# liuzuxin/FSRL

Measured on AMD Instinct MI355X. Metric: policy-updates/sec (PPO-Lagrangian update(), SafetyCarCircle-v0 shape, 256x256 MLP, 20k-step buffer), higher is better.
Workload: dtype f32; 1 GPU; configs[1] PPO-Lag update: repeat 4, clip 0.5, KL stop off, batch 256, N=20000 (20x1000), obs 8/act 2, 256x256; seeds_per_gpu=1, parallelism=independent agents x1

## Files before the change

### fsrl_amd/_lib.py

```python
import ctypes as C
import os

_HERE = os.path.dirname(os.path.abspath(__file__))
LIB_PATH = os.environ.get("FSRL_HIP_LIB") or os.path.join(_HERE, "libfsrl_hip.so")

FSRL_OK, FSRL_EINVAL, FSRL_ENOMEM, FSRL_EHIP, FSRL_ESTATE = 0, -22, -12, -5, -1
PPO_NSTATS = 11
ALGO_PPO_LAG, ALGO_TRPO_LAG, ALGO_CPO, ALGO_SAC_LAG, ALGO_FOCOPS = 0, 1, 2, 3, 4


class Config(C.Structure):
    _fields_ = [("algo", C.c_int32), ("obs_dim", C.c_int32), ("act_dim", C.c_int32),
                ("hidden", C.c_int32), ("n_critics", C.c_int32), ("env_num", C.c_int32),
                ("buffer_size", C.c_int64), ("max_action", C.c_float), ("gamma", C.c_double),
                ("gae_lambda", C.c_double), ("eps_clip", C.c_float), ("dual_clip", C.c_float),
                ("vf_coef", C.c_float), ("max_grad_norm", C.c_float), ("target_kl", C.c_float),
                ("norm_adv", C.c_int32), ("use_lagrangian", C.c_int32), ("lr", C.c_float),
                ("beta1", C.c_float), ("beta2", C.c_float), ("adam_eps", C.c_float), ("recompute_adv", C.c_int32),
                ("unbounded", C.c_int32), ("rew_norm", C.c_int32), ("value_clip", C.c_int32),
                ("hidden1", C.c_int32), ("hidden2", C.c_int32),
                ("n_hidden", C.c_int32), ("hidden_sizes", C.c_int32 * 8), ("force_layered", C.c_int32)]


class ShmEnv(C.Structure):
# ... 15 lines not shown
    _fields_ = [("actor_lr", C.c_float), ("critic_lr", C.c_float), ("alpha_lr", C.c_float), ("tau", C.c_float),
                ("alpha", C.c_float), ("target_entropy", C.c_float), ("n_step", C.c_int32),
                ("auto_alpha", C.c_int32), ("use_lagrangian", C.c_int32), ("deterministic", C.c_int32),
                ("exploration_sigma", C.c_float), ("actor_mean", C.c_int32)]


class FocopsConfig(C.Structure):
    _fields_ = [("actor_lr", C.c_float), ("critic_lr", C.c_float), ("l2_reg", C.c_float), ("delta", C.c_float),
                ("eta", C.c_float), ("tem_lambda", C.c_float), ("max_grad_norm", C.c_float)]


class CvpoConfig(C.Structure):
    _fields_ = [("actor_lr", C.c_float), ("critic_lr", C.c_float), ("tau", C.c_float), ("n_step", C.c_int32),
                ("double_critic", C.c_int32), ("sample_act_num", C.c_int32), ("estep_iter_num", C.c_int32),
                ("mstep_iter_num", C.c_int32), ("estep_kl", C.c_float), ("estep_dual_max", C.c_float),
                ("estep_dual_lr", C.c_float), ("mstep_kl_mu", C.c_float), ("mstep_kl_std", C.c_float),
                ("mstep_dual_max", C.c_float), ("mstep_dual_lr", C.c_float), ("qc_thres", C.c_double),
                ("actor_mean", C.c_int32)]


class DevEnvConfig(C.Structure):
    _fields_ = [("kind", C.c_int32), ("env_num", C.c_int32), ("obs_dim", C.c_int32), ("act_dim", C.c_int32),
                ("max_episode_steps", C.c_int32), ("seed", C.c_uint64), ("p", C.c_float * 8), ("A", C.c_void_p), ("B", C.c_void_p)]


DEVENV_POINT_CIRCLE, DEVENV_LINEAR = 0, 1

ACTOR_MEAN_DEFAULT, ACTOR_MEAN_UNBOUNDED, ACTOR_MEAN_TANH = 0, 1, 2


def actor_mean_code(unbounded):
    if unbounded is None:
        return ACTOR_MEAN_DEFAULT
    return ACTOR_MEAN_UNBOUNDED if bool(unbounded) else ACTOR_MEAN_TANH


CPO_NSTATS, TRPO_NSTATS, SAC_NSTATS, FOCOPS_NSTATS, CVPO_NSTATS = 17, 11, 10, 8, 17

_P = C.POINTER
_f, _d, _u8, _i32, _i64 = _P(C.c_float), _P(C.c_double), _P(C.c_uint8), _P(C.c_int32), _P(C.c_int64)
_ctx = C.c_void_p

SIGNATURES = {
    "fsrl_last_error": (C.c_char_p, []),
    "fsrl_config_default": (None, [_P(Config)]),
    "fsrl_mem_live": (C.c_int, [_i64, _i64, _i64, _i64]),
    "fsrl_ctx_create": (C.c_int, [C.c_int, _P(Config), _P(_ctx)]),
    "fsrl_ctx_destroy": (C.c_int, [_ctx]),
    "fsrl_sync": (C.c_int, [_ctx]),
    "fsrl_param_count": (C.c_int64, [_ctx]),
    "fsrl_params_set": (C.c_int, [_ctx, _f, C.c_int64]),
    "fsrl_params_get": (C.c_int, [_ctx, _f, C.c_int64]),
    "fsrl_grads_get": (C.c_int, [_ctx, _f, C.c_int64]),
    "fsrl_optim_reset": (C.c_int, [_ctx]),
    "fsrl_state_snapshot": (C.c_int, [_ctx]),
    "fsrl_state_restore": (C.c_int, [_ctx]),
    "fsrl_train_state_size": (C.c_int64, [_ctx, C.c_int32]),
    "fsrl_train_state_export": (C.c_int, [_ctx, C.c_int32, C.c_void_p, C.c_int64, _i64]),
    "fsrl_train_state_import": (C.c_int, [_ctx, C.c_void_p, C.c_int64]),
    "fsrl_train_state_copy": (C.c_int, [_ctx, _ctx, C.c_int32]),
    "fsrl_ret_rms_get": (C.c_int, [_ctx, _d, C.c_int32]),
    "fsrl_ret_rms_set": (C.c_int, [_ctx, _d, C.c_int32]),
    "fsrl_set_lr": (C.c_int, [_ctx, C.c_int32, C.c_float]),
    "fsrl_get_lr": (C.c_float, [_ctx, C.c_int32]),
    "fsrl_ppo_abort": (C.c_int, [_ctx]),
    "fsrl_store_push": (C.c_int, [_ctx, _i32, C.c_int32, _f, _f, _d, _d, _u8, _u8, _f, _i64, _d, _i32, _i64]),
    "fsrl_store_reset": (C.c_int, [_ctx, C.c_int]),
    "fsrl_store_len": (C.c_int64, [_ctx]),
    "fsrl_store_read": (C.c_int, [_ctx, _i64, C.c_int64, _f, _f, _d, _d, _u8, _u8, _f]),
    "fsrl_store_configure": (C.c_int, [_ctx, C.c_int64, C.c_int32]),
    "fsrl_store_geometry": (C.c_int, [_ctx, _i64, _i32]),
    "fsrl_store_version": (C.c_int, [_ctx, _P(C.c_uint64)]),
    "fsrl_store_sample0": (C.c_int, [_ctx, _i64, C.c_int64, _i64]),
    "fsrl_actor_forward": (C.c_int, [_ctx, _f, C.c_int32, _f, _f]),
    "fsrl_ppo_begin": (C.c_int, [_ctx, _d, C.c_double, C.c_int32, _i64]),
    "fsrl_ppo_pass": (C.c_int, [_ctx, _i64, C.c_uint64, _i32]),
    "fsrl_ppo_pass_result": (C.c_int, [_ctx, _i32]),
    "fsrl_ppo_end": (C.c_int, [_ctx, _f, C.c_int64, _i64]),
    "fsrl_ppo_update": (C.c_int, [_ctx, _d, C.c_double, C.c_int32, C.c_int32, _i64, C.c_uint64, _f,
                                  C.c_int64, _i64, _i32]),
    "fsrl_ppo_set_plan": (C.c_int, [_ctx, C.c_int32]),
    "fsrl_ppo_set_clip_fuse": (C.c_int, [_ctx, C.c_int32, C.c_int32]),
    "fsrl_ppo_clip_fuse_stats": (C.c_int, [_ctx, _i64, _f]),
    "fsrl_batch_get": (C.c_int, [_ctx, C.c_char_p, _f, C.c_int64]),
    "fsrl_group_create": (C.c_int, [_P(_ctx), C.c_int32, _P(_ctx)]),
    "fsrl_group_destroy": (C.c_int, [_ctx]),
    "fsrl_group_set_plan": (C.c_int, [_ctx, C.c_int32]),
    "fsrl_group_ppo_update": (C.c_int, [_ctx, _d, _d, C.c_int32, C.c_int32, _P(_i64), C.c_uint64, _P(_f), C.c_int64, _i64,
                                        _i32]),
    "fsrl_group_ppo_update_each": (C.c_int, [_ctx, _d, _d, _i32, _i32, _P(_i64), C.c_uint64, _P(_f), _i64, _i64, _i32]),
    "fsrl_group_collect_step": (C.c_int, [_ctx, _i32, _i32, _f, _f, _d, _d, _u8, _u8, _f, _i64, _d, _i32, _i64, _i32, _f, C.c_int32,
                                          C.c_int32, _f, _f, _f, _f]),
    "fsrl_group_actor_set_resident": (C.c_int, [_ctx, C.c_int32, C.c_double]),
    "fsrl_group_actor_resident_stats": (C.c_int, [_ctx, _i64]),
    "fsrl_group_actor_release": (C.c_int, [_ctx]),
    "fsrl_sac_group_create": (C.c_int, [_P(_ctx), C.c_int32, _P(_ctx)]),
    "fsrl_sac_group_destroy": (C.c_int, [_ctx]),
    "fsrl_sac_group_update": (C.c_int, [_ctx, C.c_int32, _i32, _d, _d]),
    "fsrl_cvpo_group_create": (C.c_int, [_P(_ctx), C.c_int32, _P(_ctx)]),
    "fsrl_cvpo_group_destroy": (C.c_int, [_ctx]),
    "fsrl_cvpo_group_update": (C.c_int, [_ctx, C.c_int32, _i32]),
    "fsrl_collect_group_create": (C.c_int, [_P(_ctx), C.c_int32, _P(_ctx)]),
    "fsrl_collect_group_destroy": (C.c_int, [_ctx]),
    "fsrl_collect_group_step": (C.c_int, [_ctx, _i32, _i32, _f, _f, _d, _d, _u8, _u8, _f, _i64, _d, _i32, _i64, _i32, _f, C.c_int32,
                                          C.c_int32, _f, _f, _f, _f]),
    "fsrl_collect_group_actor_set_resident": (C.c_int, [_ctx, C.c_int32, C.c_double]),
    "fsrl_collect_group_actor_resident_stats": (C.c_int, [_ctx, _i64]),
    "fsrl_collect_group_actor_release": (C.c_int, [_ctx]),
    "fsrl_group_collect_episodes": (C.c_int, [_ctx, _P(_P(ShmEnv)), _i32, _i32, _f, _i32, C.c_int32, C.c_int32, _f, _f, _i64, _d, _i32,
                                              _i32, _d, _i32, _i32, _d, _i32]),
    "fsrl_collect_episodes_group": (C.c_int, [_ctx, _P(_P(ShmEnv)), _i32, _i32, _f, _i32, C.c_int32, C.c_int32, _f, _f, _i64, _d, _i32,
                                              _i32, _d, _i32, _i32, _d, _i32]),
    "fsrl_gae_return": (C.c_int, [_ctx, _f, _f, _d, _u8, C.c_int64, C.c_double, C.c_double, _d]),
    "fsrl_nstep_return": (C.c_int, [_ctx, _d, _u8, C.c_int64, _f, _i64, C.c_int64, C.c_int64, C.c_double, C.c_int32, _d]),
    "fsrl_launch_floors": (C.c_int, [_ctx, C.c_int32, C.c_int32, _d]),
    "fsrl_tr_begin": (C.c_int, [_ctx, _P(TrConfig), _i64]),
    "fsrl_cpo_learn": (C.c_int, [_ctx, C.c_double, C.c_int32, _f]),
    "fsrl_trpo_learn": (C.c_int, [_ctx, _d, C.c_double, C.c_int32, _f]),
    "fsrl_cpo_learn_mb": (C.c_int, [_ctx, C.c_double, C.c_int32, C.c_int32, _i64, C.c_uint64, _f, C.c_int64, _i64]),
    "fsrl_trpo_learn_mb": (C.c_int, [_ctx, _d, C.c_double, C.c_int32, C.c_int32, _i64, C.c_uint64, _f, C.c_int64, _i64]),
    "fsrl_tr_linesearch_evals": (C.c_int32, [_ctx, _i32, C.c_int32]),
    "fsrl_actor_param_count": (C.c_int64, [_ctx]),
    "fsrl_tr_grad": (C.c_int, [_ctx, C.c_int32, _f, C.c_int64]),
    "fsrl_tr_hvp": (C.c_int, [_ctx, _f, _f, C.c_int64]),
    "fsrl_tr_hvp_cached": (C.c_int, [_ctx, _f, _f, C.c_int64]),
    "fsrl_tr_cg": (C.c_int, [_ctx, _f, C.c_int64, C.c_float, C.c_int32, C.c_float, _f, _i32, _f]),
    "fsrl_tr_eval": (C.c_int, [_ctx, _d]),
    "fsrl_tr_set_plan": (C.c_int, [_ctx, C.c_int32, C.c_int32, C.c_int32]),
    "fsrl_tr_set_tile_split": (C.c_int, [_ctx, C.c_int32, C.c_int32]),
    "fsrl_tr_set_co_delay": (C.c_int, [_ctx, C.c_int32, C.c_int32]),
    "fsrl_focops_init": (C.c_int, [_ctx, _P(FocopsConfig)]),
    "fsrl_focops_set_plan": (C.c_int, [_ctx, C.c_int32]),
    "fsrl_focops_set_nu": (C.c_int, [_ctx, C.c_double, C.c_double]),
    "fsrl_sac_init": (C.c_int, [_ctx, _P(SacConfig)]),
    "fsrl_sac_set_plan": (C.c_int, [_ctx, C.c_int32]),
    "fsrl_sac_param_count": (C.c_int64, [_ctx, C.c_int32]),
    "fsrl_sac_params_set": (C.c_int, [_ctx, _f, C.c_int64, _f, C.c_int64, C.c_float]),
    "fsrl_sac_params_put": (C.c_int, [_ctx, C.c_int32, _f, C.c_int64]),
    "fsrl_sac_params_get": (C.c_int, [_ctx, C.c_int32, _f, C.c_int64, _f]),
    "fsrl_sac_update": (C.c_int, [_ctx, C.c_int32, _i64, _f, _f, C.c_uint64, _d, C.c_double, _f]),
    "fsrl_actor_sample": (C.c_int, [_ctx, _f, C.c_int32, C.c_int32, C.c_uint64, _f]),
    "fsrl_collect_step": (C.c_int, [_ctx, _i32, C.c_int32, _f, _f, _d, _d, _u8, _u8, _f, _i64, _d, _i32, _i64,
                                    _f, C.c_int32, C.c_int32, C.c_int32, _f, _f, _f, _f]),
    "fsrl_collect_episodes": (C.c_int, [_ctx, _P(ShmEnv), _i32, C.c_int32, _f, C.c_int32, C.c_int32, C.c_int32, _f, _f, _i64, _d, _i32,
                                        _i32, _d, _i32, _i32]),
    "fsrl_collect_episodes_split": (C.c_int, [_ctx, _P(ShmEnv), _i32, C.c_int32, _f, C.c_int32, C.c_int32, C.c_int32, _f, _f, _i64, _d, _i32,
                                              _i32, _d, _i32, _i32]),
    "fsrl_collect_timing": (C.c_int, [_ctx, _d]),
    "fsrl_actor_set_resident": (C.c_int, [_ctx, C.c_int32, C.c_double]),
    "fsrl_actor_resident_stats": (C.c_int, [_ctx, _i64]),
    "fsrl_actor_release": (C.c_int, [_ctx]),
    "fsrl_collect_run": (C.c_int, [_ctx, _P(ShmEnv), _i32, C.c_int32, _f, _f, _f, C.c_int32, C.c_int32, _f, _f, C.c_int32, _i32, _d, _d, _d,
                                  _u8, _u8, _f]),
    "fsrl_store_sizes": (C.c_int, [_ctx, _i64, C.c_int32]),
    "fsrl_sac_stats_drain": (C.c_int64, [_ctx, _f, C.c_int64]),
    "fsrl_sac_last_sample": (C.c_int, [_ctx, _i64, _f, _f, C.c_int32]),
    "fsrl_sac_last_chain": (C.c_int, [_ctx, _i64, _u8, C.c_int32]),
    "fsrl_per_enable": (C.c_int, [_ctx, C.c_double, C.c_double, C.c_int32]),
    "fsrl_per_set_beta": (C.c_int, [_ctx, C.c_double]),
    "fsrl_per_update_weight": (C.c_int, [_ctx, _i64, _d, C.c_int64]),
    "fsrl_per_state": (C.c_int, [_ctx, _d, C.c_int64, _d, _d, _d]),
    "fsrl_per_last_weights": (C.c_int, [_ctx, _f, C.c_int32]),
    "fsrl_per_last_td": (C.c_int, [_ctx, _f, C.c_int32]),
    "fsrl_sac_actor_forward": (C.c_int, [_ctx, _f, C.c_int32, _f, _f]),
    "fsrl_cvpo_init": (C.c_int, [_ctx, _P(CvpoConfig)]),
    "fsrl_cvpo_pre_update": (C.c_int, [_ctx]),
# ... 86 lines not shown
```

### fsrl_amd/csrc/fsrl_hip.hip

```cpp
#include <hip/hip_runtime.h>

#include <climits>
#include <cstddef>
#include <cmath>
#include <cstdarg>
#include <cstdio>
#include <cstdlib>
#include <cstring>
#include <algorithm>
#include <functional>
#include <string>
#include <vector>

#include <atomic>
#include "kernels_misc.hpp"
#include "kernels_mlp.hpp"
#include "kernels_fb.hpp"
#include "kernels_fbco.hpp"
#include "kernels_wgrad2.hpp"
#include "kernels_wgrad3.hpp"
#include "kernels_layered.hpp"
#include "kernels_focops_group.hpp"
#include "resident_ring.hpp"
#include "host_decisions.hpp"
// ... 6 lines not shown
    va_start(ap, fmt);
    vsnprintf(buf, sizeof(buf), fmt, ap);
    va_end(ap);
    g_err = buf;
    return code;
}
#define HIPCHK(expr)                                                                        \
    do {                                                                                    \
        hipError_t _e = (expr);                                                             \
        if (_e != hipSuccess)                                                               \
            return fail(FSRL_EHIP, "%s failed: %s (%s:%d)", #expr, hipGetErrorString(_e),   \
                        __FILE__, __LINE__);                                                \
    } while (0)
#define CHECK_ARG(cond, ...) \
    do { if (!(cond)) return fail(FSRL_EINVAL, __VA_ARGS__); } while (0)

extern "C" const char* fsrl_last_error(void) { return g_err.c_str(); }

static inline int round_up(int x, int m) { return (x + m - 1) / m * m; }

struct TensorMap {
    int api_off, dev_off, rows, cols, dev_ld;
    int n() const { return rows * cols; }
    void to_dev(float* dev, const float* api) const {
        for (int r = 0; r < rows; ++r) memcpy(dev + dev_off + (size_t)r * dev_ld, api + api_off + (size_t)r * cols, (size_t)cols * 4);
    }
    void to_api(float* api, const float* dev) const {
        for (int r = 0; r < rows; ++r) memcpy(api + api_off + (size_t)r * cols, dev + dev_off + (size_t)r * dev_ld, (size_t)cols * 4);
    }
};

struct EnvBook {
    int64_t index = 0, size = 0, last_index = 0;
    int64_t staged = 0;
    double ep_rew = 0.0;
    int32_t ep_len = 0;
    int64_t ep_idx = 0;
};

struct Staging {
    uint8_t* h = nullptr;
    uint8_t* d = nullptr;
    int count = 0;
    hipEvent_t done = nullptr;
    bool in_flight = false;
};
static inline size_t stage_rec_bytes(int Do, int Da) { return ((size_t)24 + 4 * (size_t)(2 * Do + Da) + 7) / 8 * 8; }

struct fsrl_group;
struct fsrl_ctx {
    fsrl_config cfg{};
    Mem mem;
    fsrl_group* group = nullptr;
    struct CommState* comm = nullptr;
    int device = 0;
    hipStream_t compute = nullptr, side = nullptr;
    ModelDesc md{};
    std::vector<TensorMap> tmap;
    int h1 = 0, h2 = 0;
    int64_t n_api = 0;
    int n_dev = 0;
    int n_alloc = 0;
    float *P = nullptr, *M = nullptr, *V = nullptr, *G = nullptr;
    int64_t adam_t = 0;
    CtrlBlock* ctrl = nullptr;
    CtrlBlock* h_ctrl = nullptr;
    bool verdict_pending = false;

    int64_t sub_size = 0, maxsize = 0;
    float* mbstat = nullptr; size_t mbstat_cap = 0;
    double* d_rms = nullptr;
    double* ret64 = nullptr; int64_t ret64_cap = 0;
    int64_t alloc_rows = 0;
    int active_envs = 0;
    std::vector<EnvBook> env;
    std::vector<uint8_t> h_flags;
    StorePtrs st{};
    static constexpr int STAGE_CAP = 4096;
    Staging stage[2];
    int cur_stage = 0;
    hipEvent_t store_ready = nullptr;

    BatchPtrs b{};
    int* d_indices = nullptr; uint8_t* d_end = nullptr; int* d_seg = nullptr;
    int* h_indices = nullptr; uint8_t* h_end = nullptr; int* h_seg = nullptr;
    float *values = nullptr, *vnext = nullptr, *advs = nullptr, *rets = nullptr, *logp_old = nullptr;
    int64_t N = 0;
    int n_seg = 0;
    bool batch_ready = false;

    int batch_size = 0, mbp_max = 0, n_tiles_max = 0;
    float *A1 = nullptr, *A2 = nullptr, *D1 = nullptr, *D2 = nullptr, *DO = nullptr;
    float *obs_p = nullptr, *rd_p = nullptr;
    float *statp = nullptr, *gsq_part = nullptr;
    int *d_perm = nullptr, *h_perm = nullptr;
    int *d_mbstart = nullptr, *d_mbsize = nullptr, *h_mbplan = nullptr;
    size_t mb_cap = 0;
    std::vector<int> mb_start, mb_size;
    float* d_stats = nullptr; int64_t stats_cap = 0;
    int64_t n_steps = 0;
    int pass_index = 0;
    double lagr[FSRL_MAX_CRITICS] = {0, 0, 0, 0};
    double rescaling = 1.0;
    bool in_update = false;

    void* scratch = nullptr; size_t scratch_bytes = 0;

    bool profiling = false;
    hipEvent_t ev_a = nullptr, ev_b = nullptr, ev_c = nullptr;
    std::vector<hipEvent_t> k_ev;
    size_t k_ev_used = 0;
    double t_process_ms = 0, t_learn_ms = 0, t_fwdbwd_ms = 0, t_fwdbwd_raw_ms = 0;
    int64_t n_fwdbwd = 0;
    uint64_t rng[4] = {0x9E3779B97F4A7C15ull, 0xBF58476D1CE4E5B9ull, 0x94D049BB133111EBull, 1};
    uint64_t shuffle_rng[4] = {0xD6E8FEB86659FD93ull, 0xA0761D6478BD642Full, 0xE7037ED1A0B428DBull, 2};
    struct Parts { int stride = 0; float* p = nullptr; size_t floats = 0; } parts[3];
    float* wg_parts = nullptr;
    int n_cus = 256;
    bool wgrad_xcd = false;
    bool wgrad_stream = false;
    int wgrad_tiles = 1;
    struct FocState* foc = nullptr;
    float* mu_old = nullptr;
    float* sigma_old = nullptr;
    void* h_actor = nullptr; size_t h_actor_bytes = 0;
    int actor_k = 0; size_t actor_ob = 0, actor_mb = 0;
    unsigned* h_done = nullptr; int done_cap = 0;
    unsigned actor_seq = 0; int actor_blocks = 0;
    ResidentRing pa;
    bool pa_req = false;
    int pa_cap = 0;
    void* h_pa = nullptr;
    int probe_phase = 0, probe_wgrad_skip = 0;
    unsigned long long* probe_ts = nullptr;
    bool probe_tile16 = false;
    struct fsrl_sac_group* sac_group = nullptr;
    struct fsrl_cvpo_group* cvpo_group = nullptr;
    struct fsrl_collect_group* cgroup = nullptr;
    int tall_tiles = -1;
    bool no_fuse_adam = false;
    bool no_w2b_early = false;
    bool counted_live = false;
    int clip_fuse_mode = -1;
    int clip_fuse_limit = CLIP_FUSE_DEFAULT_TICKS;
    bool no_clip_fuse = false;
    bool clip_fuse_dead = false;
    bool clip_fuse_active = false;
    int64_t clip_fuse_fallbacks = 0, clip_fuse_steps = 0;
    unsigned clip_epoch = 0;
    unsigned long long* clip_slots = nullptr;
    float* clip_snap = nullptr;
    int64_t clip_snap_adam_t = 0;
    std::vector<std::vector<int>> clip_perms;
    bool no_xcd_pair = false;
    bool no_spin = false;
    std::vector<float> act_mu, act_sg;
    std::vector<int> perm_tmp;
    hipEvent_t perm_copied = nullptr; bool perm_in_flight = false;
    uint64_t store_version = 1;
    uint64_t joined_version = 0;
    double t_collect_env = 0.0, t_collect_act = 0.0;
    float* snap = nullptr;
    int64_t snap_adam_t = 0, snap_critic_t = 0, snap_foc_a = 0, snap_foc_c = 0; bool snap_valid = false;
    struct LayState* lay = nullptr;
    struct TrState* tr = nullptr;
    uint64_t theta_version = 1;
    void* sac = nullptr;
    struct fsrl_tap* tap = nullptr;
    struct PerState* per = nullptr;
    std::vector<struct fsrl_devenv*> devenvs;
};
static bool ctx_is_replay(const fsrl_ctx* c);
static void sac_free(fsrl_ctx* c);
static void tr_free(fsrl_ctx* c);
static void foc_free(fsrl_ctx* c);
static void tr_reset_optim(fsrl_ctx* c);
static int64_t tr_critic_steps_taken(fsrl_ctx* c);
static void tr_set_critic_steps(fsrl_ctx* c, int64_t t);
static void foc_steps(fsrl_ctx* c, int64_t* t_actor, int64_t* t_critic, bool set);
static void foc_reset_optim(fsrl_ctx* c);
static void group_detach(fsrl_ctx* c);
static void lay_free(fsrl_ctx* c);
static void lay_build_layout(fsrl_ctx* c, const int* widths, int L);
static int lay_ensure_mb(fsrl_ctx* c, int B);
static int lay_ppo_steps(fsrl_ctx* c);
struct InferArgs;
static int lay_infer(fsrl_ctx* c, const InferArgs& ia, int jobs_y, hipStream_t s);
static void comm_free(fsrl_ctx* c);
static inline bool tap_closed(const fsrl_ctx* c, int e);
static void tap_row(fsrl_ctx* c, int e, int i, const float* act, double rew, double cost, uint8_t fl);
static int tap_flush(fsrl_ctx* c, int w, const uint8_t* recs_d, int stage_rec, int k);
static void tap_ctx_gone(fsrl_ctx* c);
static void devenv_ctx_gone(fsrl_ctx* c);
static int per_ingest(fsrl_ctx* c, const uint8_t* recs_d, int rec, int k);
static int per_store_reset(fsrl_ctx* c);
static void per_free(fsrl_ctx* c);
static int focops_pass(fsrl_ctx* c, int32_t* stopped_out);
static int pass_verdict(fsrl_ctx* c, int32_t* stopped_out);

static int flush_stage(fsrl_ctx* c);
static void pactor_release(fsrl_ctx* c);
static void group_actor_release(fsrl_group* g);
static void sac_group_detach(fsrl_ctx* c);
static void cvpo_group_detach(fsrl_ctx* c);
static void collect_group_detach(fsrl_ctx* c);
static void collect_group_actor_release(struct fsrl_collect_group* g);
static int focops_group_check(fsrl_ctx* const* ctxs, int k);
struct GroupUpdate;
static int focops_group_update(GroupUpdate& u);
#define ENTER_DEV(c) do { HIPCHK(hipSetDevice((c)->device)); pactor_release(c); } while (0)

static int join_store(fsrl_ctx* c) {
    if (c->joined_version == c->store_version) return 0;
    int rc = flush_stage(c);
    if (rc) return rc;
    HIPCHK(hipEventRecord(c->store_ready, c->side));
    HIPCHK(hipStreamWaitEvent(c->compute, c->store_ready, 0));
    c->joined_version = c->store_version;
    return 0;
}

static int ensure_scratch(fsrl_ctx* c, size_t bytes) {
    HIPCHK(c->mem.regrow(c->scratch_bytes, bytes, bytes, {Mem::D(&c->scratch, bytes)}));
    return 0;
}

template <class T>
struct DevTable { T *d = nullptr, *h = nullptr; size_t cap = 0; };
template <class T>
static int table_ensure(DevTable<T>& t, size_t need, size_t grow_to, hipStream_t sync = nullptr) {
    if (need <= t.cap) return 0;
    if (sync) HIPCHK(hipStreamSynchronize(sync));
    const size_t old = t.cap * sizeof(T);
    t.cap = 0;
// ... 196 lines not shown
    if (c->sac_group) sac_group_detach(c);
    if (c->cvpo_group) cvpo_group_detach(c);
    if (c->cgroup) collect_group_detach(c);
    devenv_ctx_gone(c);
    if (c->tap) tap_ctx_gone(c);
    comm_free(c);
    tr_free(c);
    sac_free(c);
    per_free(c);
    foc_free(c);
    lay_free(c);
    c->mem.release_all();
    for (auto& st : c->stage) if (st.done) (void)hipEventDestroy(st.done);
    for (hipEvent_t e : {c->store_ready, c->ev_a, c->ev_b, c->ev_c, c->perm_copied}) if (e) (void)hipEventDestroy(e);
    for (hipEvent_t e : c->k_ev) (void)hipEventDestroy(e);
    if (c->compute) (void)hipStreamDestroy(c->compute);
    if (c->side) (void)hipStreamDestroy(c->side);
    if (c->counted_live && c->device >= 0 && c->device < 64) g_live_ctx[c->device].fetch_sub(1);
    delete c;
    return 0;
}

extern "C" int fsrl_ctx_create(int device_id, const fsrl_config* cfg, fsrl_ctx** out) {
    CHECK_ARG(cfg && out, "null argument");
    CHECK_ARG(cfg->algo == FSRL_ALGO_PPO_LAG || cfg->algo == FSRL_ALGO_SAC_LAG || cfg->algo == FSRL_ALGO_CPO ||
                  cfg->algo == FSRL_ALGO_TRPO_LAG || cfg->algo == FSRL_ALGO_FOCOPS, "unknown algo %d", cfg->algo);
    CHECK_ARG(cfg->obs_dim >= 1 && cfg->obs_dim <= FSRL_MAX_OBS, "obs_dim must be in [1,%d]", FSRL_MAX_OBS);
    CHECK_ARG(cfg->act_dim >= 1 && cfg->act_dim <= FSRL_MAX_ACT, "act_dim must be in [1,%d]", FSRL_MAX_ACT);
    CHECK_ARG(cfg->n_hidden >= 0 && cfg->n_hidden <= FSRL_MAX_HIDDEN, "n_hidden must be in [0, %d]", FSRL_MAX_HIDDEN);
    bool layered = false;
    int n_hid1 = cfg->hidden1, n_hid2 = cfg->hidden2;
    if (cfg->n_hidden > 0) {
        CHECK_ARG(cfg->hidden1 == 0 && cfg->hidden2 == 0, "give hidden_sizes[n_hidden] or hidden1 / hidden2, not both");
        for (int l = 0; l < cfg->n_hidden; ++l)
            CHECK_ARG(cfg->hidden_sizes[l] >= 1 && cfg->hidden_sizes[l] <= FSRL_MAX_WIDTH, "hidden_sizes[%d] = %d outside [1, %d]", l,
                      cfg->hidden_sizes[l], FSRL_MAX_WIDTH);
        if (cfg->n_hidden == 2 && cfg->hidden_sizes[0] <= 256 && cfg->hidden_sizes[1] <= 256 && !cfg->force_layered) {
            n_hid1 = cfg->hidden_sizes[0]; n_hid2 = cfg->hidden_sizes[1];
        } else {
            layered = true;
        }
    } else {
        CHECK_ARG(!cfg->force_layered, "force_layered needs hidden_sizes[n_hidden]");
    }
    const int h1_ = layered ? 0 : (n_hid1 > 0 ? n_hid1 : cfg->hidden), h2_ = layered ? 0 : (n_hid2 > 0 ? n_hid2 : cfg->hidden);
    if (!layered) {
        CHECK_ARG((n_hid1 > 0) == (n_hid2 > 0), "hidden1 and hidden2 are given together (0, 0 = two layers of `hidden`)");
        CHECK_ARG(h1_ >= 1 && h1_ <= 256 && h2_ >= 1 && h2_ <= 256, "hidden layer widths must be in [1, 256] (two hidden layers)");
    }
    const int Hpad_ = layered ? 0 : std::max(h1_, h2_) <= 64 ? 64 : std::max(h1_, h2_) <= 128 ? 128 : 256;
    CHECK_ARG(layered || n_hid1 == 0 || cfg->hidden == 0 || cfg->hidden == Hpad_ ,
              "hidden = %d does not fit hidden1 / hidden2 = %d / %d (leave hidden 0 or give %d)", cfg->hidden, h1_, h2_, Hpad_);
    CHECK_ARG(!layered || cfg->n_critics < 1 || cfg->n_critics > FSRL_MAX_CRITICS ||
                  (1 + cfg->n_critics) * (cfg->n_hidden + 1) + 1 <= LAY_MAX_JOBS,
              "layered context: (1 + n_critics) * (n_hidden + 1) + 1 = %d weight-gradient jobs exceed the job table of %d "
              "(n_critics = %d, n_hidden = %d)", (1 + cfg->n_critics) * (cfg->n_hidden + 1) + 1, LAY_MAX_JOBS, cfg->n_critics, cfg->n_hidden);
    CHECK_ARG(cfg->n_critics >= 1 && cfg->n_critics <= 2,
              "n_critics must be 1 or 2 (reward [+ one cost], get_metrics base_policy.py:377-382)");
    CHECK_ARG(cfg->env_num >= 1 && cfg->buffer_size >= cfg->env_num, "bad env_num/buffer_size");
    CHECK_ARG(cfg->gamma >= 0.0 && cfg->gamma <= 1.0, "discount factor should be in [0, 1].");
    CHECK_ARG(cfg->gae_lambda >= 0.0 && cfg->gae_lambda <= 1.0, "GAE lambda should be in [0, 1].");
    CHECK_ARG(cfg->dual_clip == 0.0f || cfg->dual_clip > 1.0f,
              "Dual-clip PPO parameter should greater than 1.0.");
    CHECK_ARG(cfg->buffer_size + cfg->env_num < (int64_t)INT_MAX / 2, "buffer too large for 32-bit slot ids");
    CHECK_ARG(cfg->rew_norm || !cfg->value_clip, "value clip is available only when `reward_normalization` is True");
    CHECK_ARG(!cfg->value_clip || cfg->algo == FSRL_ALGO_PPO_LAG, "value_clip is a PPO-Lagrangian option (ppo_lag.py:158-164)");
    CHECK_ARG(!cfg->rew_norm || cfg->algo != FSRL_ALGO_SAC_LAG, "reward_normalization acts on GAE returns: on-policy contexts only");
    int ndev = 0;
    HIPCHK(hipGetDeviceCount(&ndev));
    CHECK_ARG(device_id >= 0 && device_id < ndev, "device %d not present (%d devices)", device_id, ndev);
    HIPCHK(hipSetDevice(device_id));
    int n_cus_probe = 256;
    (void)hipDeviceGetAttribute(&n_cus_probe, hipDeviceAttributeMultiprocessorCount, device_id);
    fsrl_ctx* c = new fsrl_ctx();
    c->cfg = *cfg;
    c->cfg.hidden = Hpad_;
    c->h1 = h1_; c->h2 = h2_;
    c->device = device_id;
    if (device_id >= 0 && device_id < 64) { g_live_ctx[device_id].fetch_add(1); c->counted_live = true; }
    c->n_cus = n_cus_probe > 0 ? n_cus_probe : 256;
    c->probe_tile16 = getenv("FSRL_TILE16") != nullptr;
    c->no_w2b_early = getenv("FSRL_NO_W2B_EARLY") != nullptr;
    c->no_clip_fuse = getenv("FSRL_NO_CLIP_FUSE") != nullptr;
#ifdef FSRL_PROBES
    { const char* e = getenv("FSRL_DBG_PHASE"); c->probe_phase = e ? atoi(e) : 0; }
    { const char* e = getenv("FSRL_WGRAD_SKIP"); c->probe_wgrad_skip = e ? atoi(e) : 0; }
    c->no_spin = getenv("FSRL_NO_SPIN") != nullptr;
    c->no_xcd_pair = getenv("FSRL_NO_XCD_PAIR") != nullptr;
    c->no_fuse_adam = getenv("FSRL_NO_FUSE_ADAM") != nullptr;
    if (getenv("FSRL_TSTAMP")) {
        if (c->mem.dev(&c->probe_ts, 1024 * 16 * sizeof(unsigned long long)) == hipSuccess)
            (void)hipMemset(c->probe_ts, 0, 1024 * 16 * sizeof(unsigned long long));
    }
#endif
    if (layered) lay_build_layout(c, cfg->hidden_sizes, cfg->n_hidden);
    else build_layout(c);
#define TRY(expr) do { hipError_t _e = (expr); if (_e != hipSuccess) { fail(FSRL_EHIP, "%s failed: %s", #expr, hipGetErrorString(_e)); fsrl_ctx_destroy(c); return FSRL_EHIP; } } while (0)
    TRY(hipStreamCreateWithFlags(&c->compute, hipStreamNonBlocking));
    TRY(hipStreamCreateWithFlags(&c->side, hipStreamNonBlocking));
    const size_t pb = (size_t)c->n_dev * sizeof(float);
    TRY(c->mem.dev(&c->P, (size_t)c->n_alloc * sizeof(float))); TRY(hipMemsetAsync(c->P, 0, (size_t)c->n_alloc * sizeof(float), c->compute));
    TRY(c->mem.dev(&c->M, pb)); TRY(c->mem.dev(&c->V, pb)); TRY(c->mem.dev(&c->G, pb));
    TRY(hipMemsetAsync(c->M, 0, pb, c->compute)); TRY(hipMemsetAsync(c->V, 0, pb, c->compute)); TRY(hipMemsetAsync(c->G, 0, pb, c->compute));
    TRY(c->mem.dev(&c->ctrl, sizeof(CtrlBlock)));
    if (cfg->rew_norm) {
        TRY(c->mem.dev(&c->d_rms, 3 * FSRL_MAX_CRITICS * sizeof(double)));
        double init[3 * FSRL_MAX_CRITICS];
        for (int i = 0; i < FSRL_MAX_CRITICS; ++i) { init[3 * i] = 0.0; init[3 * i + 1] = 1.0; init[3 * i + 2] = 0.0; }
        TRY(hipMemcpy(c->d_rms, init, sizeof(init), hipMemcpyHostToDevice));
    }
    TRY(c->mem.pinned(&c->h_ctrl, sizeof(CtrlBlock)));
    c->sub_size = (cfg->buffer_size + cfg->env_num - 1) / cfg->env_num;
    c->maxsize = c->sub_size * cfg->env_num;
    c->alloc_rows = c->maxsize + cfg->env_num; c->active_envs = cfg->env_num;
    c->env.resize(cfg->env_num);
    c->h_flags.assign((size_t)c->alloc_rows, 0);
    const size_t ms = (size_t)c->alloc_rows;
    const int Do = cfg->obs_dim, Da = cfg->act_dim;
    TRY(c->mem.dev(&c->st.obs, ms * Do * 4)); TRY(c->mem.dev(&c->st.obs_next, ms * Do * 4));
    TRY(c->mem.dev(&c->st.act, ms * Da * 4)); TRY(c->mem.dev(&c->st.rew, ms * 8));
    TRY(c->mem.dev(&c->st.cost, ms * 8)); TRY(c->mem.dev(&c->st.flags, ms));
    TRY(c->mem.dev(&c->b.obs, ms * Do * 4)); TRY(c->mem.dev(&c->b.obs_next, ms * Do * 4));
    TRY(c->mem.dev(&c->b.act, ms * Da * 4)); TRY(c->mem.dev(&c->b.rew, ms * 8));
    TRY(c->mem.dev(&c->b.cost, ms * 8)); TRY(c->mem.dev(&c->b.flags, ms));
    TRY(c->mem.dev(&c->d_indices, ms * 4)); TRY(c->mem.dev(&c->d_end, ms)); TRY(c->mem.dev(&c->d_seg, (ms + 2) * 4));
    TRY(c->mem.pinned(&c->h_indices, ms * 4)); TRY(c->mem.pinned(&c->h_end, ms)); TRY(c->mem.pinned(&c->h_seg, (ms + 2) * 4));
    const int C = cfg->n_critics;
    TRY(c->mem.dev(&c->values, ms * C * 4)); TRY(c->mem.dev(&c->vnext, ms * C * 4));
    TRY(c->mem.dev(&c->advs, ms * C * 4)); TRY(c->mem.dev(&c->rets, ms * C * 4));
    TRY(c->mem.dev(&c->logp_old, ms * 4));
    TRY(c->mem.dev(&c->d_perm, ms * 4)); TRY(c->mem.pinned(&c->h_perm, ms * 4));
    TRY(c->mem.dev(&c->obs_p, (ms + 32) * Do * 4)); TRY(hipMemsetAsync(c->obs_p, 0, (ms + 32) * Do * 4, c->compute));
    TRY(c->mem.dev(&c->rd_p, (ms + 32) * FSRL_RD * 4)); TRY(hipMemsetAsync(c->rd_p, 0, (ms + 32) * FSRL_RD * 4, c->compute));
    TRY(hipStreamSynchronize(c->compute));
    for (auto& s : c->stage) {
        const size_t k = fsrl_ctx::STAGE_CAP;
        TRY(c->mem.pinned(&s.h, k * stage_rec_bytes(Do, Da)));
        TRY(c->mem.dev(&s.d, k * stage_rec_bytes(Do, Da)));
        TRY(hipEventCreateWithFlags(&s.done, hipEventDisableTiming));
    }
    TRY(hipEventCreateWithFlags(&c->store_ready, hipEventDisableTiming));
    TRY(hipEventCreate(&c->ev_a)); TRY(hipEventCreate(&c->ev_b)); TRY(hipEventCreate(&c->ev_c));
    TRY(hipEventCreateWithFlags(&c->perm_copied, hipEventDisableTiming));
    CtrlBlock init{INT_MAX, 0, 0.0, 0.0f, 0.0f};
    TRY(hipMemcpy(c->ctrl, &init, sizeof(init), hipMemcpyHostToDevice));
#undef TRY
    *out = c;
    return 0;
}

extern "C" int fsrl_sync(fsrl_ctx* c) {
    CHECK_ARG(c, "null ctx");
    ENTER_DEV(c);
    HIPCHK(hipStreamSynchronize(c->side));
    HIPCHK(hipStreamSynchronize(c->compute));
    return 0;
}

extern "C" int64_t fsrl_param_count(const fsrl_ctx* c) { return c ? c->n_api : 0; }

static int copy_flat(fsrl_ctx* c, float* dev, float* host_out, const float* host_in, int64_t n) {
    CHECK_ARG(n == c->n_api, "expected %lld parameters, got %lld", (long long)c->n_api, (long long)n);
    ENTER_DEV(c);
    std::vector<float> tmp((size_t)c->n_dev, 0.0f);
    if (host_in) {
        for (const TensorMap& t : c->tmap) t.to_dev(tmp.data(), host_in);
        HIPCHK(hipStreamSynchronize(c->compute));
        HIPCHK(hipMemcpy(dev, tmp.data(), (size_t)c->n_dev * 4, hipMemcpyHostToDevice));
        hipLaunchKernelGGL(w2f_sync_kernel, dim3(192), dim3(256), 0, c->compute, dev, c->md);
        HIPCHK(hipGetLastError());
    } else {
        HIPCHK(hipStreamSynchronize(c->compute));
        HIPCHK(hipMemcpy(tmp.data(), dev, (size_t)c->n_dev * 4, hipMemcpyDeviceToHost));
        for (const TensorMap& t : c->tmap) t.to_api(host_out, tmp.data());
    }
    return 0;
}

extern "C" int fsrl_params_set(fsrl_ctx* c, const float* flat, int64_t n) {
    CHECK_ARG(c && flat, "null argument");
    c->theta_version += 1;
    return copy_flat(c, c->P, nullptr, flat, n);
}
extern "C" int fsrl_params_get(fsrl_ctx* c, float* flat, int64_t n) {
    CHECK_ARG(c && flat, "null argument");
    return copy_flat(c, c->P, flat, nullptr, n);
}
extern "C" int fsrl_grads_get(fsrl_ctx* c, float* flat, int64_t n) {
    CHECK_ARG(c && flat, "null argument");
    return copy_flat(c, c->G, flat, nullptr, n);
}
extern "C" int fsrl_optim_reset(fsrl_ctx* c) {
    CHECK_ARG(c, "null ctx");
    ENTER_DEV(c);
    HIPCHK(hipStreamSynchronize(c->compute));
    HIPCHK(hipMemsetAsync(c->M, 0, (size_t)c->n_dev * 4, c->compute));
    HIPCHK(hipMemsetAsync(c->V, 0, (size_t)c->n_dev * 4, c->compute));
    HIPCHK(hipStreamSynchronize(c->compute));
    c->adam_t = 0;
    tr_reset_optim(c);
    foc_reset_optim(c);
    return 0;
}

extern "C" int fsrl_state_snapshot(fsrl_ctx* c) {
    CHECK_ARG(c, "null ctx");
    CHECK_ARG(!c->in_update, "fsrl_state_snapshot inside an update");
    CHECK_ARG(!ctx_is_replay(c), "fsrl_state_snapshot covers on-policy contexts (PPO-Lag, FOCOPS, CPO, TRPO-Lag) only");
    ENTER_DEV(c);
// ... 178 lines not shown
        for (int64_t i = eb.index; i < eb.size; ++i) idx[n++] = (int)(off + i);
        for (int64_t i = 0; i < eb.index; ++i) idx[n++] = (int)(off + i);
        if (endf) {
            for (int64_t r = first; r < n; ++r) endf[r] = c->h_flags[(size_t)idx[r]] != 0;
            if (n > first) endf[n - 1] = 1;
        }
    }
    return n;
}

extern "C" int fsrl_store_sample0(fsrl_ctx* c, int64_t* out, int64_t cap, int64_t* n_out) {
    CHECK_ARG(c && n_out, "null argument");
    const int64_t n = sample0(c, c->h_indices, nullptr);
    *n_out = n;
    if (out) {
        CHECK_ARG(cap >= n, "indices_out too small (%lld < %lld)", (long long)cap, (long long)n);
        for (int64_t i = 0; i < n; ++i) out[i] = c->h_indices[i];
    }
    return 0;
}

extern "C" int fsrl_store_read(fsrl_ctx* c, const int64_t* indices, int64_t n, float* obs_out, float* act_out,
                               double* rew_out, double* cost_out, uint8_t* terminated_out, uint8_t* truncated_out,
                               float* obs_next_out) {
    CHECK_ARG(c && (indices || n == 0), "null argument");
    CHECK_ARG(n >= 0 && n <= c->maxsize, "bad row count");
    if (n == 0) return 0;
    ENTER_DEV(c);
    int rc = join_store(c);
    if (rc) return rc;
    const size_t N = (size_t)n, Do = (size_t)c->cfg.obs_dim, Da = (size_t)c->cfg.act_dim;
    auto al = [](size_t x) { return (x + 255) / 256 * 256; };
    const size_t o_idx = 0, o_end = o_idx + al(N * 4), o_obs = o_end + al(N), o_nxt = o_obs + al(N * Do * 4),
                 o_act = o_nxt + al(N * Do * 4), o_rew = o_act + al(N * Da * 4), o_cost = o_rew + al(N * 8),
                 o_fl = o_cost + al(N * 8), total = o_fl + al(N);
    rc = ensure_scratch(c, total);
    if (rc) return rc;
    std::vector<int> idx(N);
    for (size_t i = 0; i < N; ++i) {
        CHECK_ARG(indices[i] >= 0 && indices[i] < c->maxsize, "index %lld out of range", (long long)indices[i]);
        idx[i] = (int)indices[i];
    }
    char* base = (char*)c->scratch;
    hipStream_t s = c->compute;
    HIPCHK(hipMemcpyAsync(base + o_idx, idx.data(), N * 4, hipMemcpyHostToDevice, s));
    HIPCHK(hipMemsetAsync(base + o_end, 0, N, s));
    BatchPtrs b{(float*)(base + o_obs), (float*)(base + o_nxt), (float*)(base + o_act), (double*)(base + o_rew),
                (double*)(base + o_cost), (uint8_t*)(base + o_fl)};
    const size_t work = N * (2 * Do + Da + 1);
    hipLaunchKernelGGL(batch_gather_kernel, dim3((int)std::min<size_t>(2048, (work + 255) / 256)), dim3(256), 0, s, c->st, b,
                       (const int*)(base + o_idx), (const uint8_t*)(base + o_end), (int)n, (int)Do, (int)Da);
    HIPCHK(hipGetLastError());
    std::vector<uint8_t> fl(N);
    if (obs_out) HIPCHK(hipMemcpyAsync(obs_out, b.obs, N * Do * 4, hipMemcpyDeviceToHost, s));
    if (obs_next_out) HIPCHK(hipMemcpyAsync(obs_next_out, b.obs_next, N * Do * 4, hipMemcpyDeviceToHost, s));
    if (act_out) HIPCHK(hipMemcpyAsync(act_out, b.act, N * Da * 4, hipMemcpyDeviceToHost, s));
    if (rew_out) HIPCHK(hipMemcpyAsync(rew_out, b.rew, N * 8, hipMemcpyDeviceToHost, s));
    if (cost_out) HIPCHK(hipMemcpyAsync(cost_out, b.cost, N * 8, hipMemcpyDeviceToHost, s));
    HIPCHK(hipMemcpyAsync(fl.data(), b.flags, N, hipMemcpyDeviceToHost, s));
    HIPCHK(hipStreamSynchronize(s));
    for (size_t i = 0; i < N; ++i) {
        if (terminated_out) terminated_out[i] = fl[i] & 1;
        if (truncated_out) truncated_out[i] = (fl[i] >> 1) & 1;
    }
    return 0;
}

template <typename F>
static int dispatch_H(int H, F&& f) {
    switch (H) {
        case 64: return f(std::integral_constant<int, 64>());
        case 128: return f(std::integral_constant<int, 128>());
        case 256: return f(std::integral_constant<int, 256>());
    }
    return fail(FSRL_EINVAL, "unsupported hidden width %d", H);
}

static int launch_infer(fsrl_ctx* c, const InferArgs& ia, int jobs_y, hipStream_t s) {
    const int tiles = (ia.N + 15) / 16;
    if (tiles == 0) return 0;
    if (c->lay) return lay_infer(c, ia, jobs_y, s);
    return dispatch_H(c->cfg.hidden, [&](auto hc) {
        constexpr int H = decltype(hc)::value;
        const int gx = std::min(tiles, std::max(1, c->n_cus / jobs_y));
        hipLaunchKernelGGL(mlp_infer_kernel<H>, dim3(gx, jobs_y), dim3(4 * H), 0, s, c->P, c->md, ia);
        HIPCHK(hipGetLastError());
        return 0;
    });
}

struct SacState;
static bool ctx_is_replay(const fsrl_ctx* c) { return c->cfg.algo == FSRL_ALGO_SAC_LAG; }
static int sac_actor_launch(fsrl_ctx* c, const float* h_obs, float* h_raw, int k);
static void sac_actor_finish(fsrl_ctx* c, const float* h_raw, int k, float* mu_out, float* sigma_out);
static int sac_raw_cols(const fsrl_ctx* c);
static bool sac_squashes(fsrl_ctx* c);
static bool sac_actor_resident_args(fsrl_ctx* c, const float** P, const ModelDesc** md);

struct PaLayout { unsigned long long* bell; unsigned* done; unsigned* state; float* obs; float* mu; float* sp; };
static PaLayout pa_layout(const fsrl_ctx* c) {
    char* b = (char*)c->h_pa;
    PaLayout l;
    l.bell = (unsigned long long*)b; l.done = (unsigned*)(b + 16); l.state = (unsigned*)(b + 32);
    l.obs = (float*)(b + 64);
    l.mu = l.obs + (size_t)c->pa_cap * c->cfg.obs_dim;
    l.sp = l.mu + (size_t)c->pa_cap * 2 * c->cfg.act_dim;
    return l;
}

static bool pactor_ok(const fsrl_ctx* c, int k) {
    const int blocks = std::min(PACTOR_BLOCKS, std::max(1, (c->cfg.env_num + 15) / 16));
    if (!(c->pa.on && !c->no_spin && !c->lay && !c->group && k >= 1 && k <= 16 * blocks)) return false;
    if (c->cfg.algo != FSRL_ALGO_SAC_LAG) return true;
    const float* P; const ModelDesc* md;
    return sac_actor_resident_args(const_cast<fsrl_ctx*>(c), &P, &md);
}

static void pactor_release(fsrl_ctx* c) {
    if (c->group) group_actor_release(c->group);
    if (c->cgroup) collect_group_actor_release(c->cgroup);
    rr_release(c->pa);
}

static int stream_state(hipStream_t s) {
    const hipError_t e = hipStreamQuery(s);
    if (e == hipSuccess || e == hipErrorNotReady) return e == hipSuccess ? RR_STREAM_IDLE : RR_STREAM_BUSY;
    fail(FSRL_EHIP, "the resident actor's stream: %s", hipGetErrorString(e));
    return RR_STREAM_ERROR;
}
static int rr_code(int rc, const char* what) {
    if (rc <= 0) return rc;
    if (rc == RR_ERROR) return FSRL_EHIP;
    if (rc == RR_BAD_TIMEOUT) return fail(FSRL_EINVAL, "idle_timeout_us above one second");
    return fail(FSRL_EHIP, "%s does not answer", what);
}

static int pactor_launch(void* owner, ResidentRing& r, unsigned last_seq) {
    fsrl_ctx* c = (fsrl_ctx*)owner;
    const PaLayout l = pa_layout(c);
    PActorArgs a{};
    a.obs = l.obs; a.mu_out = l.mu; a.sigma_param_out = l.sp; a.bell = l.bell; a.done = l.done; a.state = l.state;
    a.gen = r.gen; a.last_seq = last_seq; a.max_action = c->cfg.max_action;
    a.timeout_ticks = (unsigned long long)(r.idle_us * 100.0);
    r.blocks = r.tiles[0] = std::min(PACTOR_BLOCKS, std::max(1, (c->cfg.env_num + 15) / 16));
    const float* P = c->P; const ModelDesc* md = &c->md;
    if (c->cfg.algo == FSRL_ALGO_SAC_LAG) {
        if (!sac_actor_resident_args(c, &P, &md)) return fail(FSRL_ESTATE, "no fused actor network");
        a.raw_cols = sac_raw_cols(c); a.max_action = 1.0f;
    }
    const ModelDesc mdv = *md;
    return dispatch_H(c->cfg.hidden, [&](auto hc) {
        constexpr int H = decltype(hc)::value;
        if (a.raw_cols > 0) hipLaunchKernelGGL((actor_resident_kernel<H, true>), dim3(r.blocks), dim3(4 * H), 0, c->compute, P, mdv, a);
        else hipLaunchKernelGGL((actor_resident_kernel<H, false>), dim3(r.blocks), dim3(4 * H), 0, c->compute, P, mdv, a);
        HIPCHK(hipGetLastError());
        return 0;
    });
}

static int pactor_post(fsrl_ctx* c, const float* obs, int k) {
    const int Do = c->cfg.obs_dim, Da = c->cfg.act_dim;
    ResidentRing& r = c->pa;
    if (!c->h_pa) {
        const int cap = 16 * PACTOR_BLOCKS;
        const size_t bytes = 64 + ((size_t)cap * (Do + 2 * Da) + FSRL_MAX_ACT) * 4;
        HIPCHK(c->mem.regrow(c->pa_cap, cap, cap, {Mem::H(&c->h_pa, bytes)}));
        memset(c->h_pa, 0, bytes);
// ... 445 lines not shown
```

### fsrl_amd/csrc/host_decisions.hpp

```cpp
#pragma once
#include <stdint.h>
#include <algorithm>
#include <cmath>
#include <functional>
#include <queue>
#include <vector>

static constexpr float CPO_EPS = 1e-8f;
static inline bool cpo_cost_solve_skipped(float bb, float c_value) { return bb <= CPO_EPS && c_value < 0; }
struct CpoDual { int ocase; float A, B, lam, nu; };
static inline CpoDual cpo_dual_solve(float s_q, float s_r, float s_s, float c_value, float delta, float bb) {
    const float EPS = CPO_EPS;
    float A = 0.f, B = 0.f, lam, nu;
    int ocase = 4;
    if (!cpo_cost_solve_skipped(bb, c_value)) {
        A = s_q - s_r * s_r / s_s;
        B = 2.0f * delta - c_value * c_value / s_s;
        if (c_value < 0 && B < 0) ocase = 3;
        else if (c_value < 0 && B >= 0) ocase = 2;
        else if (c_value >= 0 && B >= 0) ocase = 1;
        else ocase = 0;
    }
    if (ocase == 3 || ocase == 4) {
        lam = std::sqrt(s_q / (2.0f * delta));
// ... 60 lines not shown
static inline uint64_t rotl64(uint64_t x, int k) { return (x << k) | (x >> (64 - k)); }
static inline uint64_t xoshiro_next(uint64_t* s) {
    const uint64_t result = rotl64(s[1] * 5, 7) * 9, t = s[1] << 17;
    s[2] ^= s[0]; s[3] ^= s[1]; s[1] ^= s[2]; s[0] ^= s[3]; s[2] ^= t; s[3] = rotl64(s[3], 45);
    return result;
}
enum { PERM_OK = 0, PERM_RANGE, PERM_TWICE };
struct PermFill { int code, index; long long value; };
static inline PermFill perm_fill(int* out, int n, const int64_t* perm, uint64_t* rng, uint64_t seed) {
    if (perm) {
        std::vector<uint8_t> seen((size_t)n, 0);
        for (int i = 0; i < n; ++i) {
            if (!(perm[i] >= 0 && perm[i] < n)) return {PERM_RANGE, i, (long long)perm[i]};
            if (seen[(size_t)perm[i]]) return {PERM_TWICE, i, (long long)perm[i]};
            seen[(size_t)perm[i]] = 1;
            out[i] = (int)perm[i];
        }
        return {PERM_OK, 0, 0};
    }
    if (seed) { rng[0] ^= seed; rng[1] += seed * 0x9E3779B97F4A7C15ull; }
    for (int i = 0; i < n; ++i) out[i] = i;
    for (int i = n - 1; i > 0; --i) std::swap(out[i], out[(int)(xoshiro_next(rng) % (uint64_t)(i + 1))]);
    return {PERM_OK, 0, 0};
}

struct TileSplit { int n32, n16; };
static inline TileSplit mixed_split(int64_t N, int ny, int n_cus, double rho) {
    const int max32 = (int)((N + 31) / 32);
    double best = 1e300; int best32 = 0, best16 = (int)((N + 15) / 16);
    std::vector<double> cu((size_t)std::max(n_cus, 1));
    for (int n32 = 0; n32 <= max32; ++n32) {
        const int64_t rem = N - 32 * (int64_t)n32;
        const int n16 = rem > 0 ? (int)((rem + 15) / 16) : 0;
        if (n16 > 0 && n32 == max32) continue;
        std::fill(cu.begin(), cu.end(), 0.0);
        std::priority_queue<double, std::vector<double>, std::greater<double>> pq(cu.begin(), cu.end());
        double span = 0.0;
        for (int b = 0; b < ny * n32; ++b) { const double e = pq.top() + 1.0; pq.pop(); pq.push(e); span = std::max(span, e); }
        for (int b = 0; b < ny * n16; ++b) { const double e = pq.top() + rho; pq.pop(); pq.push(e); span = std::max(span, e); }
        if (span < best - 1e-9 || (std::fabs(span - best) <= 1e-9 && n32 > best32)) { best = span; best32 = n32; best16 = n16; }
    }
    return {best32, best16};
}
static inline void co_plan(int64_t N, int n_wgs, int* n32_out, int* n16_out) {
    const int64_t tail_rows = std::min<int64_t>(N, 16 * (int64_t)(n_wgs / 2));
    const int n32 = (int)((N - tail_rows) / 32);
    const int64_t rem = N - 32 * (int64_t)n32;
    *n32_out = n32; *n16_out = (int)((rem + 15) / 16);
}
static inline void forced_split(int64_t N, int want32, int* n32_out, int* n16_out) {
    const int n32 = (int)std::min<int64_t>(want32, N / 32);
    const int64_t rem = N - 32 * (int64_t)n32;
    *n32_out = n32; *n16_out = (int)((rem + 15) / 16);
}

static constexpr int CLIP_FUSE_DEFAULT_TICKS = 5000;
static constexpr int CLIP_FUSE_MAX_OBS = 64;
struct ClipFuseFacts {
    int mode;
    bool env_off;
    bool dead;
    bool ppo_lag, layered, grouped;
    bool recompute_adv, rew_norm;
    float max_grad_norm;
    int nparts, n_cus;
    int obs_dim;
    int live_contexts;
};
static inline bool clip_fuse_update_ok(const ClipFuseFacts& f) {
    if (f.mode == 0 || f.env_off || f.dead) return false;
    if (f.mode < 0 && f.live_contexts > 1) return false;
    if (!f.ppo_lag || f.layered || f.grouped) return false;
    if (!(f.max_grad_norm > 0.0f)) return false;
    if (f.recompute_adv || f.rew_norm) return false;
    if (f.nparts > f.n_cus || f.nparts > 1024) return false;
    return f.obs_dim <= CLIP_FUSE_MAX_OBS;
}
static inline bool clip_fuse_step_ok(bool update_ok, int rows_pad) { return update_ok && rows_pad <= 512; }
static inline bool clip_fuse_must_replay(bool active, int poisoned) { return active && poisoned != 0; }
struct ClipFuseReplay { long long adam_t, n_steps; int pass_index, passes; };
static inline ClipFuseReplay clip_fuse_replay_plan(long long snap_adam_t, int passes_enqueued) {
    return {snap_adam_t, 0, 0, passes_enqueued};
}
```

### fsrl_amd/csrc/host_ppo.inc

```
static int launch_gae(fsrl_ctx* c);
static int perm_send(fsrl_ctx* c, int n);
static int clip_fuse_begin(fsrl_ctx* c);
static int perm_upload(fsrl_ctx* c, int n, const int64_t* perm, uint64_t seed) {
    c->perm_tmp.resize((size_t)n);
    const PermFill pf = perm_fill(c->perm_tmp.data(), n, perm, c->shuffle_rng, seed);
    CHECK_ARG(pf.code != PERM_RANGE, "perm[%d]=%lld out of range", pf.index, pf.value);
    CHECK_ARG(pf.code != PERM_TWICE, "perm is not a permutation: %lld appears twice", pf.value);
    return perm_send(c, n);
}
static int perm_send(fsrl_ctx* c, int n) {
    if (c->perm_in_flight) { HIPCHK(hipEventSynchronize(c->perm_copied)); c->perm_in_flight = false; }
    memcpy(c->h_perm, c->perm_tmp.data(), (size_t)n * 4);
    HIPCHK(hipMemcpyAsync(c->d_perm, c->h_perm, (size_t)n * 4, hipMemcpyHostToDevice, c->compute));
    HIPCHK(hipEventRecord(c->perm_copied, c->compute));
    c->perm_in_flight = true;
    return 0;
}

static int ensure_ppo_buffers(fsrl_ctx* c, int B) {
    const int mbp = round_up(2 * B, 32);
    if (mbp <= c->mbp_max) return 0;
    HIPCHK(hipStreamSynchronize(c->compute));
    const int H = c->cfg.hidden, nn = c->md.n_nets;
    const size_t act = (size_t)nn * mbp * H * 4;
    HIPCHK(c->mem.regrow(c->mbp_max, mbp, mbp,
                         {Mem::D(&c->A1, act), Mem::D(&c->A2, act), Mem::D(&c->D1, act), Mem::D(&c->D2, act),
                          Mem::D(&c->DO, (size_t)nn * mbp * FSRL_DOW * 4),
                          Mem::D(&c->statp, (size_t)(mbp / 4) * nn * 4 * 4),
                          Mem::D(&c->gsq_part, (size_t)std::max(wg_grid(H, nn), c->n_dev / 256 + 2) * 4)}));
    c->n_tiles_max = mbp / 16;
    return 0;
}

extern "C" int fsrl_ppo_set_plan(fsrl_ctx* c, int32_t tall_tiles) {
    CHECK_ARG(c, "null ctx");
    CHECK_ARG(tall_tiles >= -1 && tall_tiles <= 4096, "tall_tiles: -1 (automatic), 0 (none) or a count");
    c->tall_tiles = tall_tiles;
    return 0;
}

extern "C" int fsrl_ppo_begin(fsrl_ctx* c, const double* lagrangians, double rescaling,
                              int32_t batch_size, int64_t* n_out) {
    CHECK_ARG(c, "null ctx");
    CHECK_ARG(batch_size >= 1, "batch_size must be >= 1");
    CHECK_ARG(!c->in_update, "fsrl_ppo_begin called twice without fsrl_ppo_end");
    ENTER_DEV(c);
    int rc = flush_stage(c);
    if (rc) return rc;
    HIPCHK(hipEventRecord(c->store_ready, c->side));
    HIPCHK(hipStreamWaitEvent(c->compute, c->store_ready, 0));
    const int C = c->cfg.n_critics;
    for (int i = 0; i < FSRL_MAX_CRITICS; ++i) c->lagr[i] = 0.0;
    if (c->cfg.use_lagrangian && C > 1) {
        CHECK_ARG(lagrangians, "lags and values length must be equal");
        for (int i = 0; i < C - 1; ++i) c->lagr[i] = lagrangians[i];
    }
    c->rescaling = rescaling;
    c->batch_size = batch_size;
    const int64_t n = sample0(c, c->h_indices, c->h_end);
    c->N = n;
    if (n_out) *n_out = n;
    c->n_steps = 0;
    c->pass_index = 0;
    c->in_update = true;
    c->verdict_pending = false;
    c->t_fwdbwd_ms = 0; c->n_fwdbwd = 0; c->k_ev_used = 0;
    CtrlBlock init{INT_MAX, 0, 0.0, 0.0f, 0.0f};
    *c->h_ctrl = init;
    hipStream_t s = c->compute;
    HIPCHK(hipMemcpyAsync(c->ctrl, c->h_ctrl, sizeof(CtrlBlock), hipMemcpyHostToDevice, s));
    c->clip_fuse_active = false;
    c->clip_perms.clear();
    if (n == 0) { c->batch_ready = true; return 0; }
    rc = clip_fuse_begin(c);
    if (rc) return rc;
    int nseg = 0;
    c->h_seg[nseg++] = 0;
    for (int64_t i = 0; i + 1 < n; ++i) if (c->h_end[i]) c->h_seg[nseg++] = (int)i + 1;
    c->h_seg[nseg] = (int)n;
    HIPCHK(hipEventRecord(c->ev_a, s));
    HIPCHK(hipMemcpyAsync(c->d_indices, c->h_indices, (size_t)n * 4, hipMemcpyHostToDevice, s));
    HIPCHK(hipMemcpyAsync(c->d_end, c->h_end, (size_t)n, hipMemcpyHostToDevice, s));
    HIPCHK(hipMemcpyAsync(c->d_seg, c->h_seg, (size_t)(nseg + 1) * 4, hipMemcpyHostToDevice, s));
    const int Do = c->cfg.obs_dim, Da = c->cfg.act_dim;
    {
        const size_t work = (size_t)n * (2 * Do + Da + 1);
        const int blocks = (int)std::min<size_t>(2048, (work + 255) / 256);
        hipLaunchKernelGGL(batch_gather_kernel, dim3(blocks), dim3(256), 0, s, c->st, c->b, c->d_indices,
                           c->d_end, (int)n, Do, Da);
        HIPCHK(hipGetLastError());
    }
    InferArgs ia{};
    ia.obs = c->b.obs; ia.obs_next = c->b.obs_next; ia.act = c->b.act; ia.flags = c->b.flags;
    ia.values = c->values; ia.vnext = c->vnext; ia.logp_old = c->logp_old; ia.mu_out = nullptr;
    if (c->cfg.algo == FSRL_ALGO_FOCOPS) {
        if (!c->mu_old) {
            HIPCHK(c->mem.dev(&c->mu_old, (size_t)c->alloc_rows * Da * 4));
            HIPCHK(c->mem.dev(&c->sigma_old, FSRL_MAX_ACT * 4));
        }
        ia.mu_out = c->mu_old;
        HIPCHK(hipMemcpyAsync(c->sigma_old, c->P + c->md.net[0].sigma, (size_t)Da * 4, hipMemcpyDeviceToDevice, s));
    }
    ia.N = (int)n; ia.C = C; ia.max_action = c->cfg.max_action;
    rc = launch_infer(c, ia, 2 * C + 1, s);
    if (rc) return rc;
    c->n_seg = nseg;
    rc = launch_gae(c);
    if (rc) return rc;
    HIPCHK(hipEventRecord(c->ev_b, s));
    split_plan((int)n, batch_size, c->mb_start, c->mb_size);
    const int bs_rows = (int)std::min<int64_t>(batch_size, std::max<int64_t>(n, 1));
    rc = c->lay ? lay_ensure_mb(c, bs_rows) : ensure_ppo_buffers(c, bs_rows);
    if (rc) return rc;
    const size_t nmb = c->mb_start.size();
    if (nmb > c->mb_cap) {
        HIPCHK(hipStreamSynchronize(s));
        const size_t cap = nmb * 2;
        HIPCHK(c->mem.regrow(c->mb_cap, nmb, cap, {Mem::D(&c->d_mbstart, cap * 4), Mem::D(&c->d_mbsize, cap * 4), Mem::H(&c->h_mbplan, cap * 2 * 4)}));
    }
    memcpy(c->h_mbplan, c->mb_start.data(), nmb * 4);
    memcpy(c->h_mbplan + c->mb_cap, c->mb_size.data(), nmb * 4);
    HIPCHK(hipMemcpyAsync(c->d_mbstart, c->h_mbplan, nmb * 4, hipMemcpyHostToDevice, s));
    HIPCHK(hipMemcpyAsync(c->d_mbsize, c->h_mbplan + c->mb_cap, nmb * 4, hipMemcpyHostToDevice, s));
    c->batch_ready = true;
    return 0;
}


static int launch_gae(fsrl_ctx* c) {
    GaeArgs ga{};
    ga.values = c->values; ga.vnext = c->vnext; ga.rew = c->b.rew; ga.cost = c->b.cost; ga.flags = c->b.flags;
    ga.seg_start = c->d_seg; ga.advs = c->advs; ga.rets = c->rets; ga.adv64 = nullptr; ga.N = (int)c->N;
    ga.gamma = c->cfg.gamma; ga.gl = c->cfg.gamma * c->cfg.gae_lambda;
    if (c->cfg.rew_norm) {
        if (c->ret64_cap < c->N) {
            HIPCHK(hipStreamSynchronize(c->compute));
            HIPCHK(c->mem.regrow(c->ret64_cap, c->N, c->alloc_rows, {Mem::D(&c->ret64, (size_t)c->cfg.n_critics * c->alloc_rows * 8)}));
        }
        ga.rms = c->d_rms; ga.ret64 = c->ret64;
    }
    hipLaunchKernelGGL(gae_kernel, dim3(c->n_seg, c->cfg.n_critics), dim3(64), 0, c->compute, ga);
    HIPCHK(hipGetLastError());
    if (c->cfg.rew_norm) {
        hipLaunchKernelGGL(ret_rms_update_kernel, dim3(c->cfg.n_critics), dim3(1024), 0, c->compute, c->ret64, c->d_rms,
                           (int)c->N);
        HIPCHK(hipGetLastError());
    }
    return 0;
}

static int ppo_recompute_advantages(fsrl_ctx* c) {
    const int C = c->cfg.n_critics;
    InferArgs ia{};
    ia.obs = c->b.obs; ia.obs_next = c->b.obs_next; ia.act = nullptr; ia.flags = c->b.flags;
    ia.values = c->values; ia.vnext = c->vnext; ia.logp_old = nullptr; ia.mu_out = nullptr;
    ia.N = (int)c->N; ia.C = C; ia.max_action = c->cfg.max_action;
    int rc = launch_infer(c, ia, 2 * C, c->compute);
    if (rc) return rc;
    return launch_gae(c);
}

static int ensure_stats(fsrl_ctx* c, int64_t steps) {
    if (steps <= c->stats_cap) return 0;
    int64_t cap = std::max<int64_t>(steps, c->stats_cap * 2);
    cap = std::max<int64_t>(cap, 1024);
    float* nw = nullptr;
    HIPCHK(c->mem.dev(&nw, (size_t)cap * FSRL_PPO_NSTATS * 4));
    if (c->d_stats) {
        HIPCHK(hipStreamSynchronize(c->compute));
        HIPCHK(hipMemcpy(nw, c->d_stats, (size_t)c->stats_cap * FSRL_PPO_NSTATS * 4, hipMemcpyDeviceToDevice));
        HIPCHK(c->mem.release(&c->d_stats));
    }
    c->d_stats = nw;
    c->stats_cap = cap;
    return 0;
}

static int ppo_pass_prepare(fsrl_ctx* c, const int64_t* perm, uint64_t seed, const std::vector<int>* kept = nullptr) {
    const int n = (int)c->N;
    hipStream_t s = c->compute;
    const int C = c->cfg.n_critics;
    if (c->cfg.recompute_adv && c->pass_index > 0 &&
        (c->cfg.algo == FSRL_ALGO_PPO_LAG || c->cfg.algo == FSRL_ALGO_FOCOPS)) {
        int rc0 = ppo_recompute_advantages(c);
        if (rc0) return rc0;
    }
    int rc;
    if (kept) { c->perm_tmp = *kept; rc = perm_send(c, n); }
    else rc = perm_upload(c, n, perm, seed);
    if (rc) return rc;
    if (c->clip_fuse_active && !kept) c->clip_perms.push_back(c->perm_tmp);
    const int nmb = (int)c->mb_start.size();
    rc = ensure_stats(c, c->n_steps + nmb);
    if (rc) return rc;
    {
        PrepArgs pa{};
        pa.obs = c->b.obs; pa.act = c->b.act; pa.advs = c->advs; pa.rets = c->rets; pa.logp_old = c->logp_old;
        pa.perm = c->d_perm; pa.mb_start = c->d_mbstart; pa.mb_size = c->d_mbsize; pa.obs_p = c->obs_p;
        pa.rd_p = c->rd_p; pa.N = n; pa.C = C; pa.Do = c->cfg.obs_dim; pa.Da = c->cfg.act_dim;
        pa.norm_adv = c->cfg.norm_adv;
        pa.values = c->cfg.value_clip ? c->values : nullptr;
        pa.mean_old = (c->cfg.algo == FSRL_ALGO_FOCOPS) ? c->mu_old : nullptr; pa.sigma_old = c->sigma_old;
        if ((size_t)nmb > c->mbstat_cap) {
            HIPCHK(hipStreamSynchronize(s));
            HIPCHK(c->mem.regrow(c->mbstat_cap, (size_t)nmb, (size_t)nmb * 2, {Mem::D(&c->mbstat, (size_t)nmb * 2 * FSRL_MAX_CRITICS * 2 * sizeof(float))}));
        }
        pa.mbstat = c->mbstat; pa.batch = c->mb_size[0]; pa.nmb = nmb;
        if (pa.norm_adv) hipLaunchKernelGGL(ppo_adv_stats_kernel, dim3(nmb), dim3(1024), 0, s, pa);
        hipLaunchKernelGGL(ppo_permute_rows_kernel, dim3((n + 63) / 64), dim3(256), 0, s, pa);
        HIPCHK(hipGetLastError());
    }
    return 0;
}

static PpoStepArgs ppo_base_args(const fsrl_ctx* c) {
    PpoStepArgs sa{};
    sa.rescale = (float)c->rescaling;
    for (int i = 0; i < FSRL_MAX_CRITICS; ++i) sa.lam[i] = (float)c->lagr[i];
    sa.eps_clip = c->cfg.eps_clip; sa.dual_clip = c->cfg.dual_clip; sa.vf_coef = c->cfg.vf_coef;
    sa.max_action = c->cfg.max_action; sa.max_grad_norm = c->cfg.max_grad_norm; sa.target_kl = c->cfg.target_kl;
    sa.norm_adv = c->cfg.norm_adv; sa.use_lagrangian = c->cfg.use_lagrangian;
    sa.value_clip = c->cfg.value_clip;
    sa.lr = c->cfg.lr; sa.beta1 = c->cfg.beta1; sa.beta2 = c->cfg.beta2; sa.adam_eps = c->cfg.adam_eps;
    sa.one_minus_b1 = (float)(1.0 - (double)c->cfg.beta1);
    sa.one_minus_b2 = (float)(1.0 - (double)c->cfg.beta2);
    sa.kl_thresh = 1.5 * (double)c->cfg.target_kl;
    sa.pass = c->pass_index;
    sa.dbg_phase = c->probe_phase;
    sa.fuse_adam = (c->cfg.max_grad_norm <= 0.0f && !c->no_fuse_adam) ? 1 : 0;
    return sa;
}

static PpoBatchPtrs ppo_batch_ptrs(const fsrl_ctx* c) {
    PpoBatchPtrs bp{};
    bp.obs_p = c->obs_p; bp.rd_p = c->rd_p; bp.A1 = c->A1; bp.A2 = c->A2; bp.D1 = c->D1; bp.D2 = c->D2;
    bp.DO = c->DO; bp.statp = c->statp; bp.mbp_max = c->mbp_max;
    bp.ts = c->probe_ts;
    return bp;
}
// ... 94 lines not shown
                hipEvent_t e; HIPCHK(hipEventCreate(&e)); c->k_ev.push_back(e);
            }
            HIPCHK(hipEventRecord(c->k_ev[c->k_ev_used], s));
        }
        const PpoTilePlan tp = ppo_tile_plan(c, tiles, nn, 1, c->tall_tiles);
        const int n32 = tp.n32, stat_tiles = tp.rows4 ? tiles * 4 : tp.rows8 ? tiles * 2 : tiles;
        rc = dispatch_H(H, [&](auto hc) {
            constexpr int HH = decltype(hc)::value;
            sa.xcd_pair = (nn <= 4 && !c->no_xcd_pair) ? 1 : 0;
            auto fb_grid = [&](int nt) { return sa.xcd_pair ? dim3(8 * ((nt + 1) / 2)) : dim3(nt * nn); };
            const bool early = !c->no_w2b_early;
            if (tp.rows4 && early) hipLaunchKernelGGL((ppo_fwd_bwd_kernel<HH, 4, true>), fb_grid(tiles * 4), dim3(4 * HH), 0, s, c->P, c->md, bp, sa);
            else if (tp.rows4) hipLaunchKernelGGL((ppo_fwd_bwd_kernel<HH, 4>), fb_grid(tiles * 4), dim3(4 * HH), 0, s, c->P, c->md, bp, sa);
            else if (tp.rows8 && early) hipLaunchKernelGGL((ppo_fwd_bwd_kernel<HH, 8, true>), fb_grid(tiles * 2), dim3(4 * HH), 0, s, c->P, c->md, bp, sa);
            else if (tp.rows8) hipLaunchKernelGGL((ppo_fwd_bwd_kernel<HH, 8>), fb_grid(tiles * 2), dim3(4 * HH), 0, s, c->P, c->md, bp, sa);
            else if (n32 > 0) {
                if constexpr (HH >= 128)
                    hipLaunchKernelGGL((ppo_fwd_bwd_tall_kernel<HH>), dim3((tiles - n32) * nn), dim3(4 * HH), 0, s, c->P, c->md, bp, sa, n32, tiles - n32);
            } else hipLaunchKernelGGL((ppo_fwd_bwd_kernel<HH, 16>), fb_grid(tiles), dim3(4 * HH), 0, s, c->P, c->md, bp, sa);
            return 0;
        });
        if (rc) return rc;
        if (prof) {
            HIPCHK(hipEventRecord(c->k_ev[c->k_ev_used + 1], s));
            HIPCHK(hipEventRecord(c->k_ev[c->k_ev_used + 2], s));
            c->k_ev_used += 3;
        }
        const bool big = tiles * 16 > 512;
        const bool clip_step = clip_fuse_step_ok(c->clip_fuse_active, tiles * 16);
        if (clip_step) {
            c->clip_epoch += 1;
            if (c->clip_epoch == 0) c->clip_epoch = 1;
            sa.clip_epoch = c->clip_epoch; sa.clip_limit = c->clip_fuse_limit;
            c->clip_fuse_steps += 1;
        }
        if (big) {
            FbWgradArgs wa{};
            wgrad_fill_nets(wa, nn, 0, (size_t)H, (size_t)c->mbp_max, c->A1, c->A2, c->D1, c->D2, c->DO);
            wa.obs = wp.X; wa.rows = tiles * 16; wa.N = sa.mb_size;
            int nsplit = 1;
            rc = wgrad_launch<false>(c, c->md, wa, nn, c->n_dev, &nsplit);
            if (rc) return rc;
            const int nsum = (c->n_dev + 255) / 256;
            hipLaunchKernelGGL(fb_sum_parts_kernel, dim3(nsum), dim3(256), 0, s, c->G, c->wg_parts, 0, c->n_dev, nsplit, c->n_dev,
                               c->gsq_part);
            hipLaunchKernelGGL(ppo_stats_kernel, dim3(1), dim3(64), 0, s, c->md, wp, sa, stat_tiles);
            hipLaunchKernelGGL(adam_clip_kernel, dim3((c->n_dev + 4 * ADAM_NT - 1) / (4 * ADAM_NT)), dim3(ADAM_NT), 0, s, c->P, c->M,
                               c->V, c->G, c->gsq_part, nsum, c->n_dev, sa, c->ctrl, c->md);
            HIPCHK(hipGetLastError());
            continue;
        }
        rc = dispatch_H(H, [&](auto hc) {
            constexpr int HH = decltype(hc)::value;
            if (sa.fuse_adam) hipLaunchKernelGGL((ppo_wgrad_kernel<HH, false, true>), dim3(nparts), dim3(1024), 0, s, c->md, wp, tiles * 16, sa, stat_tiles);
            else if (clip_step) hipLaunchKernelGGL((ppo_wgrad_kernel<HH, false, true, true>), dim3(nparts), dim3(1024), 0, s, c->md, wp, tiles * 16, sa, stat_tiles);
            else hipLaunchKernelGGL((ppo_wgrad_kernel<HH, false, false>), dim3(nparts), dim3(1024), 0, s, c->md, wp, tiles * 16, sa, stat_tiles);
            return 0;
        });
        if (rc) return rc;
        if (!sa.fuse_adam && !clip_step)
            hipLaunchKernelGGL(adam_clip_kernel, dim3((c->n_dev + 4 * ADAM_NT - 1) / (4 * ADAM_NT)), dim3(ADAM_NT), 0, s, c->P, c->M, c->V, c->G,
                               c->gsq_part, nparts, c->n_dev, sa, c->ctrl, c->md);
        HIPCHK(hipGetLastError());
    }
    c->n_steps += nmb;
    c->pass_index += 1;
    return 0;
}

static int clip_fuse_begin(fsrl_ctx* c) {
    ClipFuseFacts f{};
    f.mode = c->clip_fuse_mode; f.env_off = c->no_clip_fuse; f.dead = c->clip_fuse_dead;
    f.ppo_lag = c->cfg.algo == FSRL_ALGO_PPO_LAG; f.layered = c->lay != nullptr; f.grouped = c->group != nullptr;
    f.recompute_adv = c->cfg.recompute_adv != 0; f.rew_norm = c->cfg.rew_norm != 0;
    f.max_grad_norm = c->cfg.max_grad_norm;
    f.nparts = c->lay ? 0 : wg_grid(c->cfg.hidden, c->md.n_nets); f.n_cus = c->n_cus; f.obs_dim = c->cfg.obs_dim;
    f.live_contexts = live_contexts_on(c->device);
    if (!clip_fuse_update_ok(f)) return 0;
    hipStream_t s = c->compute;
    if (!c->clip_slots) {
        HIPCHK(c->mem.dev(&c->clip_slots, (size_t)1024 * CLIP_SLOT_STRIDE * sizeof(unsigned long long)));
        HIPCHK(hipMemsetAsync(c->clip_slots, 0, (size_t)1024 * CLIP_SLOT_STRIDE * sizeof(unsigned long long), s));
    }
    if (!c->clip_snap) HIPCHK(c->mem.dev(&c->clip_snap, ((size_t)c->n_alloc + 2 * (size_t)c->n_dev) * 4));
    HIPCHK(hipMemcpyAsync(c->clip_snap, c->P, (size_t)c->n_alloc * 4, hipMemcpyDeviceToDevice, s));
    HIPCHK(hipMemcpyAsync(c->clip_snap + c->n_alloc, c->M, (size_t)c->n_dev * 4, hipMemcpyDeviceToDevice, s));
    HIPCHK(hipMemcpyAsync(c->clip_snap + c->n_alloc + c->n_dev, c->V, (size_t)c->n_dev * 4, hipMemcpyDeviceToDevice, s));
    c->clip_snap_adam_t = c->adam_t;
    c->clip_fuse_active = true;
    return 0;
}
static int clip_fuse_check(fsrl_ctx* c) {
    if (!clip_fuse_must_replay(c->clip_fuse_active, c->h_ctrl->poisoned)) return 0;
    hipStream_t s = c->compute;
    const ClipFuseReplay rp = clip_fuse_replay_plan(c->clip_snap_adam_t, c->pass_index);
    c->clip_fuse_active = false; c->clip_fuse_dead = true;
    c->clip_fuse_fallbacks += 1;
    HIPCHK(hipMemcpyAsync(c->P, c->clip_snap, (size_t)c->n_alloc * 4, hipMemcpyDeviceToDevice, s));
    HIPCHK(hipMemcpyAsync(c->M, c->clip_snap + c->n_alloc, (size_t)c->n_dev * 4, hipMemcpyDeviceToDevice, s));
    HIPCHK(hipMemcpyAsync(c->V, c->clip_snap + c->n_alloc + c->n_dev, (size_t)c->n_dev * 4, hipMemcpyDeviceToDevice, s));
    c->adam_t = rp.adam_t; c->n_steps = rp.n_steps; c->pass_index = rp.pass_index;
    c->k_ev_used = 0;
    CtrlBlock init{INT_MAX, 0, 0.0, 0.0f, 0.0f};
    *c->h_ctrl = init;
    HIPCHK(hipMemcpyAsync(c->ctrl, c->h_ctrl, sizeof(CtrlBlock), hipMemcpyHostToDevice, s));
    HIPCHK(hipStreamSynchronize(s));
    for (int k = 0; k < rp.passes; ++k) {
        int rc = ppo_pass_enqueue(c, nullptr, 0, &c->clip_perms[(size_t)k]);
        if (rc) return rc;
    }
    HIPCHK(hipMemcpyAsync(c->h_ctrl, c->ctrl, sizeof(CtrlBlock), hipMemcpyDeviceToHost, s));
    HIPCHK(hipStreamSynchronize(s));
    c->clip_perms.clear();
    return 0;
}
extern "C" int fsrl_ppo_set_clip_fuse(fsrl_ctx* c, int32_t mode, int32_t limit_ticks) {
    CHECK_ARG(c, "null ctx");
    CHECK_ARG(mode >= -1 && mode <= 1, "mode: -1 (automatic), 0 (off) or 1 (on)");
    CHECK_ARG(limit_ticks <= 100000000, "limit_ticks: at most 10^8 (one second)");
    CHECK_ARG(!c->in_update, "fsrl_ppo_set_clip_fuse inside an update");
    c->clip_fuse_mode = mode;
    c->clip_fuse_limit = limit_ticks < 0 ? CLIP_FUSE_DEFAULT_TICKS : limit_ticks;
    return 0;
}
extern "C" int fsrl_ppo_clip_fuse_stats(fsrl_ctx* c, int64_t* out, float* grad_norm_out) {
    CHECK_ARG(c && out, "null argument");
    if (grad_norm_out) {
        CHECK_ARG(!c->in_update, "the gradient norm is read between updates");
        ENTER_DEV(c);
        CtrlBlock cb;
        HIPCHK(hipStreamSynchronize(c->compute));
        HIPCHK(hipMemcpy(&cb, c->ctrl, sizeof(CtrlBlock), hipMemcpyDeviceToHost));
        *grad_norm_out = cb.last_grad_norm;
    }
    out[0] = (c->clip_fuse_mode != 0 && !c->no_clip_fuse && !c->clip_fuse_dead) ? 1 : 0;
    out[1] = c->clip_fuse_fallbacks; out[2] = c->clip_fuse_steps; out[3] = c->clip_fuse_active ? 1 : 0;
    return 0;
}

static int pass_verdict(fsrl_ctx* c, int32_t* stopped_out) {
    HIPCHK(hipMemcpyAsync(c->h_ctrl, c->ctrl, sizeof(CtrlBlock), hipMemcpyDeviceToHost, c->compute));
    if (!stopped_out) { c->verdict_pending = true; return 0; }
    HIPCHK(hipStreamSynchronize(c->compute));
    int rc = clip_fuse_check(c);
    if (rc) return rc;
    if (c->h_ctrl->stopped_after != INT_MAX) *stopped_out = 1;
    return 0;
}

extern "C" int fsrl_ppo_pass_result(fsrl_ctx* c, int32_t* stopped_out) {
    CHECK_ARG(c && stopped_out, "null argument");
    if (!c->in_update) return fail(FSRL_ESTATE, "fsrl_ppo_pass_result outside an update");
    ENTER_DEV(c);
    if (c->verdict_pending) {
        HIPCHK(hipStreamSynchronize(c->compute)); c->verdict_pending = false;
        int rc = clip_fuse_check(c);
        if (rc) return rc;
    }
    const bool watched = c->cfg.target_kl > 0.0f || c->cfg.algo == FSRL_ALGO_FOCOPS;
    *stopped_out = (watched && c->pass_index > 0 && c->h_ctrl->stopped_after != INT_MAX) ? 1 : 0;
    return 0;
}

extern "C" int fsrl_ppo_end(fsrl_ctx* c, float* stats_out, int64_t cap_steps, int64_t* n_steps_out) {
    CHECK_ARG(c, "null ctx");
    if (!c->in_update) return fail(FSRL_ESTATE, "fsrl_ppo_end without fsrl_ppo_begin");
    ENTER_DEV(c);
    hipStream_t s = c->compute;
    HIPCHK(hipEventRecord(c->ev_c, s));
    const bool look = c->clip_fuse_active;
    if (look) HIPCHK(hipMemcpyAsync(c->h_ctrl, c->ctrl, sizeof(CtrlBlock), hipMemcpyDeviceToHost, s));
    if (stats_out && c->n_steps > 0) {
        CHECK_ARG(cap_steps >= c->n_steps, "stats_out holds %lld steps, need %lld", (long long)cap_steps,
                  (long long)c->n_steps);
        HIPCHK(hipMemcpyAsync(stats_out, c->d_stats, (size_t)c->n_steps * FSRL_PPO_NSTATS * 4,
                              hipMemcpyDeviceToHost, s));
    }
    HIPCHK(hipStreamSynchronize(s));
    if (look) {
        c->verdict_pending = false;
        const int64_t before = c->clip_fuse_fallbacks;
        int rc = clip_fuse_check(c);
        if (rc) { c->in_update = false; return rc; }
        if (c->clip_fuse_fallbacks != before) {
            HIPCHK(hipEventRecord(c->ev_c, s));
            if (stats_out && c->n_steps > 0)
                HIPCHK(hipMemcpyAsync(stats_out, c->d_stats, (size_t)c->n_steps * FSRL_PPO_NSTATS * 4, hipMemcpyDeviceToHost, s));
            HIPCHK(hipStreamSynchronize(s));
        }
    }
    if (n_steps_out) *n_steps_out = c->n_steps;
    c->in_update = false;
    if (c->N > 0) {
        float ms = 0;
        if (hipEventElapsedTime(&ms, c->ev_a, c->ev_b) == hipSuccess) c->t_process_ms = ms;
        if (hipEventElapsedTime(&ms, c->ev_b, c->ev_c) == hipSuccess) c->t_learn_ms = ms;
        double tot = 0;
        c->t_fwdbwd_raw_ms = 0;
        for (size_t i = 0; i + 2 < c->k_ev_used; i += 3) {
            float a = 0, b = 0;
            if (hipEventElapsedTime(&a, c->k_ev[i], c->k_ev[i + 1]) == hipSuccess &&
                hipEventElapsedTime(&b, c->k_ev[i + 1], c->k_ev[i + 2]) == hipSuccess)
            { tot += (double)a - 0.5 * (double)b; c->t_fwdbwd_raw_ms += (double)a; }
        }
        c->t_fwdbwd_ms = tot;
        c->n_fwdbwd = (int64_t)(c->k_ev_used / 3);
    }
    return 0;
}

extern "C" int fsrl_ppo_update(fsrl_ctx* c, const double* lagrangians, double rescaling,
                               int32_t batch_size, int32_t repeat, const int64_t* perms, uint64_t seed,
                               float* stats_out, int64_t cap_steps, int64_t* n_steps_out,
                               int32_t* stopped_pass_out) {
    CHECK_ARG(c, "null ctx");
    CHECK_ARG(repeat >= 0, "repeat must be >= 0");
    int64_t n = 0;
    int rc = fsrl_ppo_begin(c, lagrangians, rescaling, batch_size, &n);
    if (rc) return rc;
// ... 33 lines not shown
```

### fsrl_amd/csrc/kernels_misc.hpp

```cpp
#pragma once
#include "common.hpp"

struct StorePtrs {
    float* obs;
    float* obs_next;
    float* act;
    double* rew;
    double* cost;
    uint8_t* flags;
};

__global__ void store_scatter_kernel(StorePtrs st, const uint8_t* __restrict__ recs, const int rec, int k, int Do, int Da) {
    const int per = 2 * Do + Da + 1;
    for (int e = blockIdx.x * blockDim.x + threadIdx.x; e < k * per; e += gridDim.x * blockDim.x) {
        const int row = e / per, f = e - row * per;
        const uint8_t* r = recs + (size_t)row * rec;
        const size_t dst = (size_t)*reinterpret_cast<const int*>(r + 16);
        const float* x = reinterpret_cast<const float*>(r + 24);
        if (f < Do) st.obs[dst * Do + f] = x[f];
        else if (f < 2 * Do) st.obs_next[dst * Do + (f - Do)] = x[f];
        else if (f < 2 * Do + Da) st.act[dst * Da + (f - 2 * Do)] = x[f];
        else {
            st.rew[dst] = *reinterpret_cast<const double*>(r);
            st.cost[dst] = *reinterpret_cast<const double*>(r + 8);
            st.flags[dst] = (uint8_t)*reinterpret_cast<const uint32_t*>(r + 20);
        }
    }
}

struct BatchPtrs {
    float* obs; float* obs_next; float* act; double* rew; double* cost; uint8_t* flags;
};

__global__ void batch_gather_kernel(StorePtrs st, BatchPtrs b, const int* __restrict__ indices,
                                    const uint8_t* __restrict__ end_flag, int n, int Do, int Da) {
    const int per = 2 * Do + Da + 1;
    for (size_t e = (size_t)blockIdx.x * blockDim.x + threadIdx.x; e < (size_t)n * per;
         e += (size_t)gridDim.x * blockDim.x) {
        const int row = (int)(e / per), f = (int)(e - (size_t)row * per);
        const size_t src = (size_t)indices[row];
        if (f < Do) b.obs[(size_t)row * Do + f] = st.obs[src * Do + f];
        else if (f < 2 * Do) b.obs_next[(size_t)row * Do + (f - Do)] = st.obs_next[src * Do + (f - Do)];
        else if (f < 2 * Do + Da) b.act[(size_t)row * Da + (f - 2 * Do)] = st.act[src * Da + (f - 2 * Do)];
        else {
            b.rew[row] = st.rew[src];
            b.cost[row] = st.cost[src];
            b.flags[row] = (uint8_t)((st.flags[src] & 3) | (end_flag[row] ? 4 : 0));
        }
    }
}

struct GaeArgs {
    const float* values;
    const float* vnext;
    const double* rew;
    const double* cost;
    const uint8_t* flags;
    const int* seg_start;
    float* advs;
    float* rets;
    double* adv64;
    int N;
    double gamma, gl;
    const double* rms;
    double* ret64;
};
#define FSRL_RMS_EPS 1e-8

__device__ __forceinline__ double readlane_f64(double x, int l) {
    const int lo = __builtin_amdgcn_readlane(__double2loint(x), l);
    const int hi = __builtin_amdgcn_readlane(__double2hiint(x), l);
    return __hiloint2double(hi, lo);
}

__global__ __launch_bounds__(64) void gae_kernel(const GaeArgs a) {
#pragma clang fp contract(off)
    const int seg = blockIdx.x, c = blockIdx.y, lane = threadIdx.x;
    const int s = a.seg_start[seg], e = a.seg_start[seg + 1];
    const float* __restrict__ v = a.values + (size_t)c * a.N;
    const float* __restrict__ vn = a.vnext + (size_t)c * a.N;
    const double* __restrict__ met = (c == 0) ? a.rew : a.cost;
    const double scale = a.rms ? sqrt(a.rms[3 * c + 1] + FSRL_RMS_EPS) : 1.0;
    double g = 0.0;
    for (int base = e - 64; base > s - 64; base -= 64) {
        const int idx = base + lane;
        const bool ok = idx >= s;
        double delta = 0.0, disc = 0.0, vv = 0.0;
        if (ok) {
            vv = (double)v[idx];
            double vnx = (double)vn[idx];
            if (a.rms) { vv = vv * scale; vnx = vnx * scale; }
            const double t0 = vnx * a.gamma;
            const double t1 = met[idx] + t0;
            delta = t1 - vv;
            disc = (1.0 - ((a.flags[idx] & 4) ? 1.0 : 0.0)) * a.gl;
        }
        double res = 0.0;
#pragma unroll
        for (int t = 63; t >= 0; --t) {
            const double dt = readlane_f64(delta, t);
            const double ct = readlane_f64(disc, t);
            const double prod = ct * g;
            g = dt + prod;
            if (lane == t) res = g;
        }
        if (ok) {
            const size_t o = (size_t)c * a.N + idx;
            a.advs[o] = (float)res;
            double ret = res + vv;
            if (a.rms) { ret = ret / scale; a.ret64[o] = ret; }
            a.rets[o] = (float)ret;
            if (a.adv64) a.adv64[o] = res;
        }
    }
}

__global__ __launch_bounds__(1024) void ret_rms_update_kernel(const double* __restrict__ ret64, double* __restrict__ rms,
                                                              const int N) {
    __shared__ double sh[16];
    __shared__ double bc;
    const int c = blockIdx.x, tid = threadIdx.x;
    const double* __restrict__ x = ret64 + (size_t)c * N;
    auto block_sum = [&](double v) {
        for (int o = 32; o > 0; o >>= 1) v += __shfl_down(v, o, 64);
        if ((tid & 63) == 0) sh[tid >> 6] = v;
        __syncthreads();
        if (tid == 0) { double t = 0.0; for (int w = 0; w < 16; ++w) t += sh[w]; bc = t; }
        __syncthreads();
        const double r = bc;
        __syncthreads();
// ... 227 lines not shown
```

### fsrl_amd/csrc/kernels_mlp.hpp

```cpp
#pragma once
#include <type_traits>
#include "common.hpp"

__host__ __device__ constexpr int tile_rows(int R) { return R > 16 ? R : 16; }

template <int H, int ROWS = 16>
struct TileSmem {
    static constexpr int LD = H + 4;
    static constexpr int XK = (ROWS > 16) ? 64 : FSRL_MAX_OBS;
    float xT[XK * ROWS];
    float h1[ROWS * LD];
    float h2[ROWS * LD];
    float d2[ROWS * LD];
    float out[ROWS * FSRL_MAX_ACT];
    float dout[ROWS * FSRL_DOW];
    float rd[ROWS * FSRL_RD];
    float st[ROWS * 4];
    float w3[FSRL_MAX_ACT * H];
    float b1[H], b2[H], b3[FSRL_MAX_ACT], sig[FSRL_MAX_ACT];
    float w1[H * FSRL_W1_LDS];
};

template <int H>
struct TileGeom {
    static constexpr int NT = 4 * H;
    static constexpr int WAVES = H / 16;
};

template <int H>
struct FwdW2Frag {
    f32x4 b[H / 16];
    __device__ __forceinline__ void load(const float* __restrict__ W2f, int wave, int lane) {
        const float* base = W2f + ((size_t)wave * (H / 16) * 64 + lane) * 4;
#pragma unroll
        for (int kc = 0; kc < H / 16; ++kc) b[kc] = *reinterpret_cast<const f32x4*>(base + kc * 256);
    }
    __device__ __forceinline__ void load_buf(const float* __restrict__ W2f, int wave, int lane) {
        const Wg3Buf bw = wg3_buf_here(W2f);
        const unsigned frag0 = (unsigned)wave * (unsigned)(H / 16) * 256u;
#pragma unroll
        for (int kc = 0; kc < H / 16; ++kc) b[kc] = wg3_ld4s(bw, 4u * (unsigned)lane, frag0 + 256u * (unsigned)kc);
    }
};

template <int H, int ROWS = 16>
struct TileStage {
    static constexpr int NT = TileGeom<H>::NT;
    static constexpr int NX = (ROWS * TileSmem<H, ROWS>::XK + NT - 1) / NT;
    static constexpr int NR = (ROWS * FSRL_RD + NT - 1) / NT;
    float xv[NX], w3v[4], w1v[4], rdv[NR], b1v, b2v, b3v, sgv;

    __device__ __forceinline__ void issue(const float* __restrict__ P, const NetOff no, const int Do,
                                          const int Da, const float* __restrict__ x,
                                          const float* __restrict__ rd, const int n_valid,
                                          const int tid) {
        const int nx = n_valid * Do;
#pragma unroll
        for (int u = 0; u < NX; ++u) {
            const int e = tid + u * NT;
            const float v = x[min(e, max(nx - 1, 0))];
            xv[u] = (e < nx) ? v : 0.0f;
        }
        const int n3 = no.out * H, n1 = (Do <= FSRL_W1_LDS) ? H * Do : 0;
#pragma unroll
        for (int u = 0; u < 4; ++u) {
            const int e = tid + u * NT;
            const float a = P[no.W3 + min(e, n3 - 1)];
            const float b = P[no.W1 + min(e, max(n1 - 1, 0))];
            w3v[u] = (e < n3) ? a : 0.0f;
            w1v[u] = (e < n1) ? b : 0.0f;
        }
        const int nr = n_valid * FSRL_RD;
#pragma unroll
        for (int u = 0; u < NR; ++u) {
            const int e = tid + u * NT;
            const float v = (rd != nullptr) ? rd[min(e, max(nr - 1, 0))] : 0.0f;
            rdv[u] = (rd != nullptr && e < nr) ? v : 0.0f;
        }
        const float t1 = P[no.b1 + min(tid, H - 1)], t2 = P[no.b2 + min(tid, H - 1)];
        const float t3 = P[no.b3 + min(tid, no.out - 1)];
        const float t4 = P[max(no.sigma, 0) + min(tid, Da - 1)];
        b1v = (tid < H) ? t1 : 0.0f;
        b2v = (tid < H) ? t2 : 0.0f;
        b3v = (tid < no.out) ? t3 : 0.0f;
        sgv = (no.sigma >= 0 && tid < Da) ? t4 : 0.0f;
// ... 182 lines not shown
            for (int r = 0; r < 4; ++r) {
                sm.h2[r * LD + j] = fmaxf(acc[r] + bias, 0.0f);
                if constexpr (R == 8) sm.h2[(4 + r) * LD + j] = fmaxf(acc8[r] + bias, 0.0f);
            }
        }
        hook.phase(1);
    } else {
        f32x4 acc = {0.f, 0.f, 0.f, 0.f}, acc2 = {0.f, 0.f, 0.f, 0.f};
        const float* arow = &sm.h1[li * LD + 4 * q];
#pragma unroll
        for (int kc = 0; kc < H / 16; ++kc) {
            const f32x4 a = *reinterpret_cast<const f32x4*>(arow + 16 * kc);
#pragma unroll
            for (int s = 0; s < 4; ++s) acc = mfma_16x16x4(a[s], wf.b[kc][s], acc);
            if constexpr (R == 32) {
                const f32x4 a2 = *reinterpret_cast<const f32x4*>(arow + 16 * LD + 16 * kc);
#pragma unroll
                for (int s = 0; s < 4; ++s) acc2 = mfma_16x16x4(a2[s], wf.b[kc][s], acc2);
            }
        }
        const int j = wave * 16 + li;
        const float bias = sm.b2[j];
#pragma unroll
        for (int r = 0; r < 4; ++r) {
            sm.h2[(4 * q + r) * LD + j] = fmaxf(acc[r] + bias, 0.0f);
            if constexpr (R == 32) sm.h2[(16 + 4 * q + r) * LD + j] = fmaxf(acc2[r] + bias, 0.0f);
        }
    }
    __syncthreads();
    FSRL_TS(ts, 5);
    if constexpr (R < 16) hook.phase(2);

    if constexpr (WIDE_HEAD && R <= 16) {
        if (no.out > 4) {
            const f32x4 av = *reinterpret_cast<const f32x4*>(&sm.h2[li * LD + 16 * wave + 4 * q]);
            const f32x4 wv = *reinterpret_cast<const f32x4*>(&sm.w3[li * H + 16 * wave + 4 * q]);
            const bool on = li < no.out;
            f32x4 acc = {0.f, 0.f, 0.f, 0.f};
#pragma unroll
            for (int s2 = 0; s2 < 4; ++s2) acc = mfma_16x16x4(av[s2], on ? wv[s2] : 0.0f, acc);
            float* __restrict__ part = sm.d2;
#pragma unroll
            for (int r = 0; r < 4; ++r) part[(wave * 16 + 4 * q + r) * 16 + li] = acc[r];
            __syncthreads();
            if (tid < 16 * R) {
                const int i = tid >> 4, o = tid & 15;
                float t = 0.0f;
#pragma unroll
                for (int w = 0; w < WAVES; ++w) t += part[(w * 16 + i) * 16 + o];
                if (o < no.out) sm.out[i * FSRL_MAX_ACT + o] = t + sm.b3[o];
            }
            __syncthreads();
            return;
        }
    }
    for (int idx = wave; idx < R * no.out; idx += WAVES) {
        const int i = idx / no.out, o = idx - i * no.out;
        const float* w3 = &sm.w3[o * H];
        float s = 0.0f;
#pragma unroll
        for (int k = lane; k < H; k += 64) s = fmaf(sm.h2[i * LD + k], w3[k], s);
        s = wave_sum(s);
        if (lane == 0) sm.out[i * FSRL_MAX_ACT + o] = s + sm.b3[o];
    }
    __syncthreads();
}

struct InferArgs {
    const float* obs;
    const float* obs_next;
    const float* act;
    const uint8_t* flags;
    float* values;
    float* vnext;
    float* logp_old;
    float* mu_out;
    int N, C;
    float max_action;
    float* raw_out;
    int raw_cols;
    float* sigma_param_out;
    unsigned* done;
    unsigned seq;
};

#define LOG_SQRT_2PI 0.9189385332046727f

template <int H>
__global__ __launch_bounds__(4 * H) void mlp_infer_kernel(const float* __restrict__ P,
                                                         const ModelDesc md, const InferArgs a) {
    __shared__ TileSmem<H> sm;
    constexpr int NT = TileGeom<H>::NT;
    constexpr int NX = TileStage<H>::NX;
    const int tid = threadIdx.x;
    const int job = blockIdx.y;
    const int C = a.C;
    const bool is_actor = (job == 2 * C);
    const int net = is_actor ? 0 : 1 + (C > 0 ? job % C : 0);
    const bool use_next = (!is_actor) && job >= C;
    const NetOff no = md.net[net];
    const int Do = md.Do;
    const int n_tiles = (a.N + 15) >> 4;
    const unsigned magic = div_magic(Do);
    const float* __restrict__ X = use_next ? a.obs_next : a.obs;
    int tile = blockIdx.x;
    int row0 = tile * 16;
    int n_valid = min(16, a.N - row0);
    TileStage<H> stg;
    stg.issue(P, no, Do, md.Da, X + (size_t)row0 * Do, nullptr, n_valid, tid);
    FwdW2Frag<H> wf;
    wf.load(P + no.W2f, tid >> 6, tid & 63);
    stg.commit(sm, no, Do, tid);
    while (true) {
        const int ntile = tile + gridDim.x;
        const int nrow0 = ntile * 16, nn_valid = min(16, a.N - nrow0);
        float xn[NX];
        if (ntile < n_tiles) {
#pragma unroll
            for (int u = 0; u < NX; ++u) {
                const int e = tid + u * NT;
                xn[u] = (e < nn_valid * Do) ? X[(size_t)nrow0 * Do + e] : 0.0f;
            }
        }
        __syncthreads();
        tile_forward<H>(sm, P, no, Do, tid, wf);
        if (a.sigma_param_out && is_actor && tile == 0 && tid < md.Da && no.sigma >= 0) a.sigma_param_out[tid] = sm.sig[tid];
        if (a.raw_out) {
            for (int e = tid; e < n_valid * a.raw_cols; e += NT) {
                const int i = e / a.raw_cols, o = e - i * a.raw_cols;
                a.raw_out[(size_t)(row0 + i) * a.raw_cols + o] = sm.out[i * FSRL_MAX_ACT + o];
            }
        } else if (tid < n_valid) {
            const int r = row0 + tid;
            if (!is_actor) {
                float v = sm.out[tid * FSRL_MAX_ACT];
                const int c = (C > 0) ? job % C : 0;
                if (use_next) {
                    if (a.flags[r] & 1) v = 0.0f;
                    a.vnext[(size_t)c * a.N + r] = v;
                } else {
                    a.values[(size_t)c * a.N + r] = v;
                }
            } else {
                float logp = 0.0f;
                for (int d = 0; d < md.Da; ++d) {
                    const float x = sm.out[tid * FSRL_MAX_ACT + d];
                    const float mu = md.unbounded ? x : a.max_action * tanhf(x);
                    const float sig = expf(sm.sig[d]);
                    if (a.mu_out) a.mu_out[(size_t)r * md.Da + d] = mu;
                    if (a.act) {
                        const float diff = a.act[(size_t)r * md.Da + d] - mu;
                        logp += -(diff * diff) / (2.0f * sig * sig) - logf(sig) - LOG_SQRT_2PI;
                    }
                }
                if (a.logp_old) a.logp_old[r] = logp;
            }
        }
        if (ntile >= n_tiles) break;
        __syncthreads();
#pragma unroll
        for (int u = 0; u < NX; ++u) {
            const int e = tid + u * NT;
            if (e < 16 * Do) { const int i = div_by_magic((unsigned)e, magic), k = e - i * Do; sm.xT[k * 16 + i] = xn[u]; }
        }
        tile = ntile; row0 = nrow0; n_valid = nn_valid;
    }
    if (a.done) {
        if (tid < min(NT, max(256, (16 * a.raw_cols + 63) & ~63))) __atomic_thread_fence(__ATOMIC_RELEASE);
        __syncthreads();
        if (tid == 0) __hip_atomic_store(a.done + blockIdx.x, a.seq, __ATOMIC_RELAXED, __HIP_MEMORY_SCOPE_SYSTEM);
    }
}

#define PACTOR_BLOCKS 4
struct PActorArgs {
    const float* obs;
    float* mu_out;
    float* sigma_param_out;
    const unsigned long long* bell;
    unsigned* done;
    unsigned* state;
    unsigned gen, last_seq;
    unsigned long long timeout_ticks;
    float max_action;
    int raw_cols;
};
#define PACTOR_EXIT 0xFFFFFFFFu

template <int H, bool RAW>
__global__ __launch_bounds__(4 * H) void actor_resident_kernel(const float* __restrict__ P, const ModelDesc md, const PActorArgs a) {
    __shared__ TileSmem<H> sm;
    __shared__ unsigned k_s, seq_s;
    __shared__ unsigned last_s;
    constexpr int NT = TileGeom<H>::NT;
    constexpr int NX = TileStage<H>::NX;
    const int tid = threadIdx.x, blk = blockIdx.x;
    const NetOff no = md.net[0];
    const int Do = md.Do;
    const unsigned magic = div_magic(Do);
    TileStage<H> stg;
    stg.issue(P, no, Do, md.Da, P, nullptr, 0, tid);
    FwdW2Frag<H> wf;
    wf.load(P + no.W2f, tid >> 6, tid & 63);
    stg.commit(sm, no, Do, tid);
    if (tid == 0) last_s = a.last_seq;
    for (;;) {
        __syncthreads();
        if (tid == 0) {
            const unsigned long long t0 = wall_clock64();
            const unsigned last = last_s;
            unsigned long long v;
            unsigned polls = 0;
            for (;;) {
                v = __hip_atomic_load(a.bell, __ATOMIC_RELAXED, __HIP_MEMORY_SCOPE_SYSTEM);
                if ((unsigned)v != last) break;
                if (wall_clock64() - t0 > a.timeout_ticks || ++polls > (1u << 26)) { v = (unsigned long long)PACTOR_EXIT << 32; break; }
                __builtin_amdgcn_s_sleep(1);
            }
            __atomic_thread_fence(__ATOMIC_ACQUIRE);
            k_s = (unsigned)(v >> 32); seq_s = (unsigned)v;
            last_s = (unsigned)v;
        }
        __syncthreads();
        const unsigned k = k_s;
// ... 1062 lines not shown
```

### fsrl_amd/engine.py

```python
import ctypes as C
from dataclasses import dataclass
from typing import Optional, Sequence

import numpy as np

from . import _lib

_f32p, _f64p = C.POINTER(C.c_float), C.POINTER(C.c_double)
_u8p, _i32p, _i64p = C.POINTER(C.c_uint8), C.POINTER(C.c_int32), C.POINTER(C.c_int64)


def _ptr(a, t):
    return a.ctypes.data_as(t) if a is not None else None


def mem_live():
    v = [C.c_int64(0) for _ in range(4)]
    _lib.check(_lib.load().fsrl_mem_live(*[C.byref(x) for x in v]))
    return dict(zip(("dev_blocks", "dev_bytes", "pinned_blocks", "pinned_bytes"), (x.value for x in v)))


@dataclass
class EngineConfig:
    obs_dim: int = 8
# ... 392 lines not shown
        ep_rew, ep_len = np.zeros(max(int(n_episode), 1), np.float64), np.zeros(max(int(n_episode), 1), np.int32)
        _lib.check(fn(
            self._ctx, h, int(n_episode), int(bool(deterministic)), int(bound_method), _ptr(lo, _f32p), _ptr(hi, _f32p),
            int(max_steps_per_launch), C.byref(steps), C.byref(cost), C.byref(nt), C.byref(ntr), _ptr(ep_rew, _f64p),
            _ptr(ep_len, _i32p), C.byref(nep), C.byref(nl)))
        k = nep.value
        return dict(steps=int(steps.value), total_cost=float(cost.value), terminated=int(nt.value), truncated=int(ntr.value),
                    ep_rews=ep_rew[:k], ep_lens=ep_len[:k], launches=int(nl.value))

    def actor_set_resident(self, on=True, idle_timeout_us=0.0):
        _lib.check(self.lib.fsrl_actor_set_resident(self._ctx, int(bool(on)), float(idle_timeout_us)))

    def actor_release(self):
        self.lib.fsrl_actor_release(self._ctx)

    def actor_resident_stats(self):
        out = np.zeros(3, np.int64)
        _lib.check(self.lib.fsrl_actor_resident_stats(self._ctx, _ptr(out, _i64p)))
        return dict(launches=int(out[0]), requests=int(out[1]), live=bool(out[2]))

    def store_sizes(self, n=None):
        n = self.cfg.env_num if n is None else int(n)
        out = np.empty(n, np.int64)
        _lib.check(self.lib.fsrl_store_sizes(self._ctx, _ptr(out, _i64p), n))
        return out

    def focops_init(self, actor_lr=5e-4, critic_lr=1e-3, l2_reg=1e-3, delta=0.02, eta=0.02, tem_lambda=0.95,
                    max_grad_norm=0.5):
        cfg = _lib.FocopsConfig(actor_lr, critic_lr, l2_reg, delta, eta, tem_lambda, float(max_grad_norm or 0.0))
        _lib.check(self.lib.fsrl_focops_init(self._ctx, C.byref(cfg)))

    def focops_set_plan(self, four_launch: int = 0):
        _lib.check(self.lib.fsrl_focops_set_plan(self._ctx, int(four_launch)))

    def focops_update(self, nu, nu_loss, batch_size, repeat, perms=None, seed=0):
        _lib.check(self.lib.fsrl_focops_set_nu(self._ctx, float(nu), float(nu_loss)))
        stats, stopped = self.ppo_update([0.0], 1.0, batch_size, repeat, perms=perms, seed=seed)
        return stats[:, :_lib.FOCOPS_NSTATS], stopped

    def ppo_begin(self, lagrangians: Sequence[float], rescaling: float, batch_size: int) -> int:
        lag = np.ascontiguousarray(lagrangians, np.float64).reshape(-1)
        n = C.c_int64()
        _lib.check(self.lib.fsrl_ppo_begin(self._ctx, _ptr(lag, _f64p) if lag.size else None,
                                           float(rescaling), int(batch_size), C.byref(n)))
        self._n = n.value
        return n.value

    def ppo_pass(self, perm=None, seed: int = 0, wait: bool = True) -> bool:
        stopped = C.c_int32()
        if perm is not None:
            perm = np.ascontiguousarray(perm, np.int64)
            assert perm.size == self._n, "permutation length != batch length"
        _lib.check(self.lib.fsrl_ppo_pass(self._ctx, _ptr(perm, _i64p), int(seed), C.byref(stopped) if wait else None))
        return bool(stopped.value)

    def ppo_pass_result(self) -> bool:
        stopped = C.c_int32()
        _lib.check(self.lib.fsrl_ppo_pass_result(self._ctx, C.byref(stopped)))
        return bool(stopped.value)

    def ppo_end(self):
        n = C.c_int64()
        _lib.check(self.lib.fsrl_ppo_end(self._ctx, None, 0, C.byref(n)))
        return n.value

    def ppo_end_stats(self, max_steps: int):
        n = C.c_int64()
        out = np.empty((max(max_steps, 1), _lib.PPO_NSTATS), np.float32)
        _lib.check(self.lib.fsrl_ppo_end(self._ctx, _ptr(out, _f32p), out.shape[0], C.byref(n)))
        return out[:n.value]

    def ppo_set_plan(self, tall_tiles: int = -1):
        _lib.check(self.lib.fsrl_ppo_set_plan(self._ctx, int(tall_tiles)))

    def ppo_set_clip_fuse(self, mode: int = -1, limit_ticks: int = -1):
        _lib.check(self.lib.fsrl_ppo_set_clip_fuse(self._ctx, int(mode), int(limit_ticks)))

    def ppo_clip_fuse_stats(self):
        out = (C.c_int64 * 4)()
        gn = C.c_float()
        _lib.check(self.lib.fsrl_ppo_clip_fuse_stats(self._ctx, out, C.byref(gn)))
        return dict(available=bool(out[0]), fallbacks=int(out[1]), steps=int(out[2]), last_update_fused=bool(out[3]),
                    grad_norm=np.float32(gn.value))

    def ppo_update(self, lagrangians, rescaling, batch_size, repeat, perms=None, seed=0):
        n = self.ppo_begin(lagrangians, rescaling, batch_size)
        stopped_pass = -1
        steps_per_pass = max(1, -(-n // max(batch_size, 1)))
        try:
            for k in range(repeat):
                if self.ppo_pass(None if perms is None else perms[k], seed + k if seed else 0):
                    stopped_pass = k
                    break
            stats = self.ppo_end_stats(steps_per_pass * max(repeat, 1))
        except BaseException:
            self.ppo_abort()
            raise
        return stats, stopped_pass

    def batch_get(self, which: str):
        n = self._n
        cols = 1 if which == "logp_old" else self.cfg.n_critics
        out = np.empty((n, cols), np.float32)
        _lib.check(self.lib.fsrl_batch_get(self._ctx, which.encode(), _ptr(out, _f32p), out.size))
        return out[:, 0] if which == "logp_old" else out

    def gae_return(self, v, v_next, rew, end_flag, gamma, gae_lambda):
        v = np.ascontiguousarray(v, np.float32); v_next = np.ascontiguousarray(v_next, np.float32)
        rew = np.ascontiguousarray(rew, np.float64)
        end = np.ascontiguousarray(end_flag).astype(np.uint8)
        out = np.empty(rew.size, np.float64)
        _lib.check(self.lib.fsrl_gae_return(self._ctx, _ptr(v, _f32p), _ptr(v_next, _f32p),
                                            _ptr(rew, _f64p), _ptr(end, _u8p), rew.size, float(gamma),
                                            float(gae_lambda), _ptr(out, _f64p)))
        return out

    def launch_floors(self, mb_rows=256, iters=200):
        out = np.zeros(4, np.float64)
        _lib.check(self.lib.fsrl_launch_floors(self._ctx, int(mb_rows), int(iters), _ptr(out, _f64p)))
        return dict(zip(("fwdbwd", "wgrad", "adam", "triple"), out.tolist()))

    def nstep_return(self, metric, end_flag, target_q, indices, gamma, n_step):
        metric = np.ascontiguousarray(metric, np.float64)
        end = np.ascontiguousarray(end_flag).astype(np.uint8)
        tq = np.ascontiguousarray(target_q, np.float32)
        shape = tq.shape
        bsz = shape[0] if tq.ndim else 0
        tq2 = tq.reshape(bsz, -1) if bsz else tq.reshape(0, 1)
        idx = np.ascontiguousarray(indices, np.int64).reshape(int(n_step), bsz) if n_step >= 1 else np.zeros((0, bsz), np.int64)
        out = np.empty(tq2.shape, np.float64)
        _lib.check(self.lib.fsrl_nstep_return(self._ctx, _ptr(metric, _f64p), _ptr(end, _u8p), metric.size,
                                              _ptr(tq2, _f32p), _ptr(idx, _i64p), bsz, tq2.shape[1], float(gamma),
                                              int(n_step), _ptr(out, _f64p)))
        return out.reshape(shape)

    def tr_begin(self, target_kl=0.01, backtrack_coeff=0.8, damping=0.1, l2_reg=0.0, critic_lr=1e-3,
                 max_backtracks=10, optim_critic_iters=10, cg_iters=10, norm_adv=True,
                 cost_limit=float("inf")) -> int:
        cfg = _lib.TrConfig(target_kl, backtrack_coeff, damping, l2_reg, critic_lr, max_backtracks,
                            optim_critic_iters, cg_iters, int(norm_adv),
                            cost_limit if np.isfinite(cost_limit) else 1e300)
        n = C.c_int64()
        _lib.check(self.lib.fsrl_tr_begin(self._ctx, C.byref(cfg), C.byref(n)))
        self._n = n.value
        return n.value

    @property
    def n_actor_params(self) -> int:
        return int(self.lib.fsrl_actor_param_count(self._ctx))

    def tr_linesearch_evals(self, cap=64):
        out = np.zeros(cap, np.int32)
        n = int(self.lib.fsrl_tr_linesearch_evals(self._ctx, _ptr(out, _i32p), cap))
        return out[:n]

    def tr_grad(self, which: int):
        out = np.empty(self.n_actor_params, np.float32)
        _lib.check(self.lib.fsrl_tr_grad(self._ctx, int(which), _ptr(out, _f32p), out.size))
        return out

    def tr_hvp(self, v):
        v = np.ascontiguousarray(v, np.float32)
        out = np.empty_like(v)
        _lib.check(self.lib.fsrl_tr_hvp(self._ctx, _ptr(v, _f32p), _ptr(out, _f32p), v.size))
        return out

# ... 630 lines not shown
```

### include/fsrl_hip.h

```cpp
#ifndef FSRL_HIP_H
#define FSRL_HIP_H

#include <stdint.h>

#ifdef __cplusplus
extern "C" {
#endif

#define FSRL_OK 0
#define FSRL_EINVAL (-22)
#define FSRL_ENOMEM (-12)
#define FSRL_EHIP (-5)
#define FSRL_ESTATE (-1)

#define FSRL_ALGO_PPO_LAG 0
#define FSRL_ALGO_TRPO_LAG 1
#define FSRL_ALGO_CPO 2
#define FSRL_ALGO_SAC_LAG 3
#define FSRL_ALGO_FOCOPS 4

#define FSRL_MAX_CRITICS 4
#define FSRL_MAX_HIDDEN 8
#define FSRL_MAX_WIDTH 4096
#define FSRL_PPO_NSTATS 11
// ... 49 lines not shown
int64_t fsrl_train_state_size(fsrl_ctx* ctx, int32_t with_store);
int fsrl_train_state_export(fsrl_ctx* ctx, int32_t with_store, void* out, int64_t cap, int64_t* written);
int fsrl_train_state_import(fsrl_ctx* ctx, const void* blob, int64_t n);
int fsrl_train_state_copy(fsrl_ctx* dst, fsrl_ctx* src, int32_t with_store);
int fsrl_ret_rms_get(fsrl_ctx* ctx, double* out, int32_t n);
int fsrl_ret_rms_set(fsrl_ctx* ctx, const double* in, int32_t n);
int fsrl_set_lr(fsrl_ctx* ctx, int32_t group, float lr);
float fsrl_get_lr(const fsrl_ctx* ctx, int32_t group);

int fsrl_store_push(fsrl_ctx* ctx, const int32_t* env_ids, int32_t k, const float* obs,
                    const float* act, const double* rew, const double* cost,
                    const uint8_t* terminated, const uint8_t* truncated,
                    const float* obs_next, int64_t* ptr_out, double* ep_rew_out,
                    int32_t* ep_len_out, int64_t* ep_idx_out);
int fsrl_store_reset(fsrl_ctx* ctx, int keep_statistics);
int64_t fsrl_store_len(const fsrl_ctx* ctx);
int fsrl_store_read(fsrl_ctx* ctx, const int64_t* indices, int64_t n, float* obs_out, float* act_out, double* rew_out,
                    double* cost_out, uint8_t* terminated_out, uint8_t* truncated_out, float* obs_next_out);
int fsrl_store_configure(fsrl_ctx* ctx, int64_t total_size, int32_t buffer_num);
int fsrl_store_geometry(const fsrl_ctx* ctx, int64_t* sub_size_out, int32_t* buffer_num_out);
int fsrl_store_version(const fsrl_ctx* ctx, uint64_t* version_out);
int fsrl_store_sample0(fsrl_ctx* ctx, int64_t* indices_out, int64_t cap, int64_t* n_out);

int fsrl_actor_forward(fsrl_ctx* ctx, const float* obs, int32_t k, float* mu_out,
                       float* sigma_out);
int fsrl_actor_sample(fsrl_ctx* ctx, const float* obs, int32_t k, int32_t deterministic, uint64_t seed,
                      float* act_out);
int fsrl_collect_step(fsrl_ctx* ctx, const int32_t* env_ids, int32_t k, const float* obs, const float* act,
                      const double* rew, const double* cost, const uint8_t* terminated, const uint8_t* truncated,
                      const float* obs_next, int64_t* ptr_out, double* ep_rew_out, int32_t* ep_len_out,
                      int64_t* ep_idx_out, const float* obs_act, int32_t k_act, int32_t deterministic,
                      int32_t bound_method, const float* act_low, const float* act_high, float* act_out,
                      float* env_act_out);
typedef struct fsrl_shm_env {
    float* obs;
    float* act;
    double* rew; double* cost;
    uint8_t* term; uint8_t* trunc; uint8_t* active;
    uint32_t* hs;
    uint32_t* want;
    const int32_t* owner;
    const int32_t* lane_of_worker;
    int32_t env_num, obs_dim, act_dim, workers, n_lanes;
    uint32_t gen[2];
    uint32_t spin;
    const uint32_t* err;
    const int32_t* pids;
} fsrl_shm_env;
int fsrl_collect_run(fsrl_ctx* ctx, fsrl_shm_env* env, const int32_t* ready, int32_t n, float* obs, float* act,
                     float* env_act, int32_t deterministic, int32_t bound_method, const float* act_low,
                     const float* act_high, int32_t max_steps, int32_t* steps_out, double* cost_sum_out, double* rew_out,
                     double* cost_out, uint8_t* term_out, uint8_t* trunc_out, float* obs_next_out);
int fsrl_collect_episodes(fsrl_ctx* ctx, fsrl_shm_env* env, const int32_t* ready, int32_t n, const float* obs, int32_t n_episode,
                          int32_t deterministic, int32_t bound_method, const float* act_low, const float* act_high,
                          int64_t* steps_out, double* total_cost_out, int32_t* term_count_out, int32_t* trunc_count_out,
                          double* ep_rew_out, int32_t* ep_len_out, int32_t* episodes_out);

int fsrl_collect_episodes_split(fsrl_ctx* ctx, fsrl_shm_env* env, const int32_t* ready, int32_t n, const float* obs, int32_t n_episode,
                                int32_t deterministic, int32_t bound_method, const float* act_low, const float* act_high,
                                int64_t* steps_out, double* total_cost_out, int32_t* term_count_out, int32_t* trunc_count_out,
                                double* ep_rew_out, int32_t* ep_len_out, int32_t* episodes_out);
int fsrl_collect_timing(fsrl_ctx* ctx, double* out2);
int fsrl_actor_set_resident(fsrl_ctx* ctx, int32_t on, double idle_timeout_us);
int fsrl_actor_resident_stats(fsrl_ctx* ctx, int64_t* out3);
int fsrl_actor_release(fsrl_ctx* ctx);

int fsrl_store_sizes(const fsrl_ctx* ctx, int64_t* sizes_out, int32_t n);

int fsrl_ppo_begin(fsrl_ctx* ctx, const double* lagrangians, double rescaling,
                   int32_t batch_size, int64_t* n_out);
int fsrl_ppo_pass(fsrl_ctx* ctx, const int64_t* perm, uint64_t seed, int32_t* stopped_out);
int fsrl_ppo_pass_result(fsrl_ctx* ctx, int32_t* stopped_out);
int fsrl_ppo_end(fsrl_ctx* ctx, float* stats_out, int64_t cap_steps, int64_t* n_steps_out);
int fsrl_ppo_abort(fsrl_ctx* ctx);
int fsrl_ppo_update(fsrl_ctx* ctx, const double* lagrangians, double rescaling,
                    int32_t batch_size, int32_t repeat, const int64_t* perms, uint64_t seed,
                    float* stats_out, int64_t cap_steps, int64_t* n_steps_out,
                    int32_t* stopped_pass_out);

int fsrl_ppo_set_plan(fsrl_ctx* ctx, int32_t tall_tiles);

int fsrl_ppo_set_clip_fuse(fsrl_ctx* ctx, int32_t mode, int32_t limit_ticks);
int fsrl_ppo_clip_fuse_stats(fsrl_ctx* ctx, int64_t* out, float* grad_norm_out);

typedef struct fsrl_group fsrl_group;
int fsrl_group_create(fsrl_ctx** ctxs, int32_t k, fsrl_group** out);
int fsrl_group_destroy(fsrl_group* group);
int fsrl_group_set_plan(fsrl_group* group, int32_t tall_tiles);
int fsrl_group_ppo_update(fsrl_group* group, const double* lagrangians, const double* rescaling, int32_t batch_size,
                          int32_t repeat, const int64_t* const* perms, uint64_t seed, float* const* stats_out,
                          int64_t cap_steps, int64_t* n_steps_out, int32_t* stopped_pass_out);
int fsrl_group_ppo_update_each(fsrl_group* group, const double* lagrangians, const double* rescaling, const int32_t* batch_sizes,
                               const int32_t* repeats, const int64_t* const* perms, uint64_t seed, float* const* stats_out,
                               const int64_t* cap_steps, int64_t* n_steps_out, int32_t* stopped_pass_out);
int fsrl_group_collect_step(fsrl_group* group, const int32_t* k, const int32_t* env_ids, const float* obs, const float* act,
                            const double* rew, const double* cost, const uint8_t* terminated, const uint8_t* truncated,
                            const float* obs_next, int64_t* ptr_out, double* ep_rew_out, int32_t* ep_len_out,
                            int64_t* ep_idx_out, const int32_t* k_act, const float* obs_act, int32_t deterministic,
                            int32_t bound_method, const float* act_low, const float* act_high, float* act_out,
                            float* env_act_out);
int fsrl_group_actor_set_resident(fsrl_group* group, int32_t on, double idle_timeout_us);
int fsrl_group_actor_resident_stats(fsrl_group* group, int64_t* out3);
int fsrl_group_actor_release(fsrl_group* group);

int fsrl_batch_get(fsrl_ctx* ctx, const char* which, float* out, int64_t cap);

int fsrl_gae_return(fsrl_ctx* ctx, const float* v, const float* v_next, const double* rew,
                    const uint8_t* end_flag, int64_t n, double gamma, double gae_lambda,
                    double* adv_out);

int fsrl_nstep_return(fsrl_ctx* ctx, const double* metric, const uint8_t* end_flag, int64_t len,
                      const float* target_q, const int64_t* indices, int64_t bsz, int64_t q, double gamma,
                      int32_t n_step, double* out);

typedef struct fsrl_tr_config {
    float target_kl;
    float backtrack_coeff;
    float damping;
    float l2_reg;
    float critic_lr;
    int32_t max_backtracks;
    int32_t optim_critic_iters;
    int32_t cg_iters;
    int32_t norm_adv;
    double cost_limit;
} fsrl_tr_config;

#define FSRL_CPO_NSTATS 17
#define FSRL_TRPO_NSTATS 11

int fsrl_tr_begin(fsrl_ctx* ctx, const fsrl_tr_config* cfg, int64_t* n_out);
int fsrl_cpo_learn(fsrl_ctx* ctx, double ave_cost_return, int32_t repeat, float* stats_out);
int fsrl_trpo_learn(fsrl_ctx* ctx, const double* lagrangians, double rescaling, int32_t repeat,
                    float* stats_out);
int fsrl_cpo_learn_mb(fsrl_ctx* ctx, double ave_cost_return, int32_t repeat, int32_t batch_size, const int64_t* perms,
                      uint64_t seed, float* stats_out, int64_t cap_rows, int64_t* n_rows_out);
int fsrl_trpo_learn_mb(fsrl_ctx* ctx, const double* lagrangians, double rescaling, int32_t repeat, int32_t batch_size,
                       const int64_t* perms, uint64_t seed, float* stats_out, int64_t cap_rows, int64_t* n_rows_out);
int32_t fsrl_tr_linesearch_evals(fsrl_ctx* ctx, int32_t* out, int32_t cap);
int64_t fsrl_actor_param_count(const fsrl_ctx* ctx);
int fsrl_tr_grad(fsrl_ctx* ctx, int32_t which, float* out, int64_t n);
int fsrl_tr_hvp(fsrl_ctx* ctx, const float* v, float* out, int64_t n);
int fsrl_tr_hvp_cached(fsrl_ctx* ctx, const float* v, float* out, int64_t n);
int fsrl_tr_cg(fsrl_ctx* ctx, const float* rhs, int64_t n, float damping, int32_t nsteps, float tol, float* x_out,
               int32_t* iters_out, float* rs_out);
int fsrl_tr_eval(fsrl_ctx* ctx, double* stats8);
int fsrl_tr_set_plan(fsrl_ctx* ctx, int32_t tile_rows, int32_t hvp, int32_t wgrad);
int fsrl_tr_set_tile_split(fsrl_ctx* ctx, int32_t n32_tile, int32_t n32_hvp);
int fsrl_tr_set_co_delay(fsrl_ctx* ctx, int32_t tile_periods, int32_t hvp_periods);

typedef struct fsrl_focops_config {
    float actor_lr, critic_lr;
    float l2_reg;
    float delta;
    float eta;
    float tem_lambda;
    float max_grad_norm;
} fsrl_focops_config;
#define FSRL_FOCOPS_NSTATS 8
int fsrl_focops_init(fsrl_ctx* ctx, const fsrl_focops_config* cfg);
int fsrl_focops_set_plan(fsrl_ctx* ctx, int32_t four_launch);
int fsrl_focops_set_nu(fsrl_ctx* ctx, double nu, double nu_loss);

typedef struct fsrl_sac_config {
    float actor_lr, critic_lr, alpha_lr;
    float tau;
// ... 174 lines not shown
```

Baseline: 141.7 updates/s.

## Reuse critic values for next-obs rows and coalesce begin-time uploads

The gather kernel now also marks rows whose obs_next equals the next row's obs and compacts the non-matching rows into a miss list. The value-inference kernel then evaluates next-state critics only on those miss rows and fills the rest of vnext from the current-state values, rebalancing blocks between the jobs. It also packs the control block, indices, segments and minibatch plan into one pinned upload block sent with a single copy, and stores P/M/V contiguously so clip-fuse snapshot and restore each need one copy. This drops most next-state critic forwards and several small H2D copies, at the cost of an atomic-compacted list, gathered loads and a more complex block mapping.

```diff
diff --git a/fsrl_amd/_lib.py b/fsrl_amd/_lib.py
--- a/fsrl_amd/_lib.py
+++ b/fsrl_amd/_lib.py
@@ -121,6 +121,7 @@
     "fsrl_ppo_set_plan": (C.c_int, [_ctx, C.c_int32]),
     "fsrl_ppo_set_clip_fuse": (C.c_int, [_ctx, C.c_int32, C.c_int32]),
     "fsrl_ppo_clip_fuse_stats": (C.c_int, [_ctx, _i64, _f]),
+    "fsrl_ppo_process_stats": (C.c_int, [_ctx, _i64]),
     "fsrl_batch_get": (C.c_int, [_ctx, C.c_char_p, _f, C.c_int64]),
     "fsrl_group_create": (C.c_int, [_P(_ctx), C.c_int32, _P(_ctx)]),
     "fsrl_group_destroy": (C.c_int, [_ctx]),
diff --git a/fsrl_amd/csrc/fsrl_hip.hip b/fsrl_amd/csrc/fsrl_hip.hip
--- a/fsrl_amd/csrc/fsrl_hip.hip
+++ b/fsrl_amd/csrc/fsrl_hip.hip
@@ -112,8 +112,14 @@
     hipEvent_t store_ready = nullptr;
 
     BatchPtrs b{};
+    char *d_up = nullptr, *h_up = nullptr;
     int* d_indices = nullptr; uint8_t* d_end = nullptr; int* d_seg = nullptr;
     int* h_indices = nullptr; uint8_t* h_end = nullptr; int* h_seg = nullptr;
+    uint8_t* next_same = nullptr;
+    int* miss_list = nullptr;
+    int* miss_count = nullptr;
+    bool no_vnext_reuse = false;
+    bool vnext_reuse_active = false;
     float *values = nullptr, *vnext = nullptr, *advs = nullptr, *rets = nullptr, *logp_old = nullptr;
     int64_t N = 0;
     int n_seg = 0;
@@ -124,8 +130,7 @@
     float *obs_p = nullptr, *rd_p = nullptr;
     float *statp = nullptr, *gsq_part = nullptr;
     int *d_perm = nullptr, *h_perm = nullptr;
-    int *d_mbstart = nullptr, *d_mbsize = nullptr, *h_mbplan = nullptr;
-    size_t mb_cap = 0;
+    int *d_mbstart = nullptr, *d_mbsize = nullptr;
     std::vector<int> mb_start, mb_size;
     float* d_stats = nullptr; int64_t stats_cap = 0;
     int64_t n_steps = 0;
@@ -179,7 +184,8 @@
     int64_t clip_fuse_fallbacks = 0, clip_fuse_steps = 0;
     unsigned clip_epoch = 0;
     unsigned long long* clip_slots = nullptr;
-    float* clip_snap = nullptr;
+    char* clip_snap = nullptr;
+    char* pmv = nullptr; size_t pmv_bytes = 0;
     int64_t clip_snap_adam_t = 0;
     std::vector<std::vector<int>> clip_perms;
     bool no_xcd_pair = false;
@@ -542,6 +548,7 @@
     c->probe_tile16 = getenv("FSRL_TILE16") != nullptr;
     c->no_w2b_early = getenv("FSRL_NO_W2B_EARLY") != nullptr;
     c->no_clip_fuse = getenv("FSRL_NO_CLIP_FUSE") != nullptr;
+    c->no_vnext_reuse = getenv("FSRL_NO_VNEXT_REUSE") != nullptr;
 #ifdef FSRL_PROBES
     { const char* e = getenv("FSRL_DBG_PHASE"); c->probe_phase = e ? atoi(e) : 0; }
     { const char* e = getenv("FSRL_WGRAD_SKIP"); c->probe_wgrad_skip = e ? atoi(e) : 0; }
@@ -559,17 +566,21 @@
     TRY(hipStreamCreateWithFlags(&c->compute, hipStreamNonBlocking));
     TRY(hipStreamCreateWithFlags(&c->side, hipStreamNonBlocking));
     const size_t pb = (size_t)c->n_dev * sizeof(float);
-    TRY(c->mem.dev(&c->P, (size_t)c->n_alloc * sizeof(float))); TRY(hipMemsetAsync(c->P, 0, (size_t)c->n_alloc * sizeof(float), c->compute));
-    TRY(c->mem.dev(&c->M, pb)); TRY(c->mem.dev(&c->V, pb)); TRY(c->mem.dev(&c->G, pb));
-    TRY(hipMemsetAsync(c->M, 0, pb, c->compute)); TRY(hipMemsetAsync(c->V, 0, pb, c->compute)); TRY(hipMemsetAsync(c->G, 0, pb, c->compute));
-    TRY(c->mem.dev(&c->ctrl, sizeof(CtrlBlock)));
+    {
+        auto al = [](size_t x) { return (x + 255) / 256 * 256; };
+        const size_t pbytes = al((size_t)c->n_alloc * sizeof(float));
+        c->pmv_bytes = pbytes + 2 * al(pb);
+        TRY(c->mem.dev(&c->pmv, c->pmv_bytes)); TRY(hipMemsetAsync(c->pmv, 0, c->pmv_bytes, c->compute));
+        c->P = reinterpret_cast<float*>(c->pmv); c->M = reinterpret_cast<float*>(c->pmv + pbytes);
+        c->V = reinterpret_cast<float*>(c->pmv + pbytes + al(pb));
+    }
+    TRY(c->mem.dev(&c->G, pb)); TRY(hipMemsetAsync(c->G, 0, pb, c->compute));
     if (cfg->rew_norm) {
         TRY(c->mem.dev(&c->d_rms, 3 * FSRL_MAX_CRITICS * sizeof(double)));
         double init[3 * FSRL_MAX_CRITICS];
         for (int i = 0; i < FSRL_MAX_CRITICS; ++i) { init[3 * i] = 0.0; init[3 * i + 1] = 1.0; init[3 * i + 2] = 0.0; }
         TRY(hipMemcpy(c->d_rms, init, sizeof(init), hipMemcpyHostToDevice));
     }
-    TRY(c->mem.pinned(&c->h_ctrl, sizeof(CtrlBlock)));
     c->sub_size = (cfg->buffer_size + cfg->env_num - 1) / cfg->env_num;
     c->maxsize = c->sub_size * cfg->env_num;
     c->alloc_rows = c->maxsize + cfg->env_num; c->active_envs = cfg->env_num;
@@ -583,8 +594,18 @@
     TRY(c->mem.dev(&c->b.obs, ms * Do * 4)); TRY(c->mem.dev(&c->b.obs_next, ms * Do * 4));
     TRY(c->mem.dev(&c->b.act, ms * Da * 4)); TRY(c->mem.dev(&c->b.rew, ms * 8));
     TRY(c->mem.dev(&c->b.cost, ms * 8)); TRY(c->mem.dev(&c->b.flags, ms));
-    TRY(c->mem.dev(&c->d_indices, ms * 4)); TRY(c->mem.dev(&c->d_end, ms)); TRY(c->mem.dev(&c->d_seg, (ms + 2) * 4));
-    TRY(c->mem.pinned(&c->h_indices, ms * 4)); TRY(c->mem.pinned(&c->h_end, ms)); TRY(c->mem.pinned(&c->h_seg, (ms + 2) * 4));
+    static_assert(sizeof(CtrlBlock) <= 64, "the control block leads the upload block: 64 bytes");
+    TRY(c->mem.dev(&c->d_up, upload_capacity(ms))); TRY(c->mem.pinned(&c->h_up, upload_capacity(ms)));
+    TRY(hipMemsetAsync(c->d_up, 0, upload_capacity(ms), c->compute));
+    memset(c->h_up, 0, upload_capacity(ms));
+    {
+        const UploadLayout u = upload_layout(ms, ms, ms);
+        c->ctrl = (CtrlBlock*)(c->d_up + u.ctrl); c->h_ctrl = (CtrlBlock*)(c->h_up + u.ctrl);
+        c->miss_count = (int*)(c->d_up + u.miss_count);
+        c->d_indices = (int*)(c->d_up + u.indices); c->h_indices = (int*)(c->h_up + u.indices);
+    }
+    TRY(c->mem.pinned(&c->h_end, ms)); TRY(c->mem.pinned(&c->h_seg, (ms + 2) * 4));
+    TRY(c->mem.dev(&c->next_same, ms)); TRY(c->mem.dev(&c->miss_list, ms * 4));
     const int C = cfg->n_critics;
     TRY(c->mem.dev(&c->values, ms * C * 4)); TRY(c->mem.dev(&c->vnext, ms * C * 4));
     TRY(c->mem.dev(&c->advs, ms * C * 4)); TRY(c->mem.dev(&c->rets, ms * C * 4));
@@ -929,7 +950,7 @@
     if (c->lay) return lay_infer(c, ia, jobs_y, s);
     return dispatch_H(c->cfg.hidden, [&](auto hc) {
         constexpr int H = decltype(hc)::value;
-        const int gx = std::min(tiles, std::max(1, c->n_cus / jobs_y));
+        const int gx = infer_grid_x(tiles, c->n_cus, jobs_y);
         hipLaunchKernelGGL(mlp_infer_kernel<H>, dim3(gx, jobs_y), dim3(4 * H), 0, s, c->P, c->md, ia);
         HIPCHK(hipGetLastError());
         return 0;
diff --git a/fsrl_amd/csrc/host_decisions.hpp b/fsrl_amd/csrc/host_decisions.hpp
--- a/fsrl_amd/csrc/host_decisions.hpp
+++ b/fsrl_amd/csrc/host_decisions.hpp
@@ -166,3 +166,51 @@
 static inline ClipFuseReplay clip_fuse_replay_plan(long long snap_adam_t, int passes_enqueued) {
     return {snap_adam_t, 0, 0, passes_enqueued};
 }
+
+#if defined(__HIPCC__)
+#define FSRL_HD __host__ __device__
+#else
+#define FSRL_HD
+#endif
+static inline int infer_grid_x(int tiles, int n_cus, int jobs_y) { return std::min(tiles, std::max(1, n_cus / jobs_y)); }
+struct InferSplit { int bn, bf, equal; };
+FSRL_HD static inline InferSplit infer_split(int gx, int jobs_y, int C, int n_tiles, int miss_tiles) {
+    const int F = jobs_y - C, T = gx * jobs_y;
+    InferSplit s{0, 0, 0};
+    if (miss_tiles > 0) {
+        const long long den = (long long)F * n_tiles + (long long)C * miss_tiles;
+        long long bn = ((long long)T * miss_tiles + den - 1) / den;
+        if (bn > gx) bn = gx;
+        if (bn > miss_tiles) bn = miss_tiles;
+        if (bn < 1) bn = 1;
+        s.bn = (int)bn;
+    }
+    if (s.bn == gx) { s.bf = gx; s.equal = 1; return s; }
+    s.bf = (T - C * s.bn) / F;
+    if (s.bf > n_tiles) s.bf = n_tiles;
+    return s;
+}
+static inline int next_same_count(const uint32_t* obs, const uint32_t* obs_next, int n, int Do) {
+    int same = 0;
+    for (int r = 0; r + 1 < n; ++r) {
+        bool eq = true;
+        for (int k = 0; k < Do && eq; ++k) eq = obs_next[(size_t)r * Do + k] == obs[(size_t)(r + 1) * Do + k];
+        same += eq ? 1 : 0;
+    }
+    return same;
+}
+
+struct UploadLayout { size_t ctrl, miss_count, indices, end, seg, mb_start, mb_size, total; };
+static constexpr size_t UPLOAD_HEAD = 128;
+static inline size_t upload_align(size_t x) { return (x + 63) / 64 * 64; }
+static inline UploadLayout upload_layout(size_t n, size_t n_seg, size_t n_mb) {
+    UploadLayout u{};
+    u.ctrl = 0; u.miss_count = 64; u.indices = UPLOAD_HEAD;
+    u.end = u.indices + upload_align(n * 4);
+    u.seg = u.end + upload_align(n);
+    u.mb_start = u.seg + upload_align((n_seg + 1) * 4);
+    u.mb_size = u.mb_start + upload_align(n_mb * 4);
+    u.total = u.mb_size + upload_align(n_mb * 4);
+    return u;
+}
+static inline size_t upload_capacity(size_t rows) { return upload_layout(rows, rows, rows).total; }
diff --git a/fsrl_amd/csrc/host_ppo.inc b/fsrl_amd/csrc/host_ppo.inc
--- a/fsrl_amd/csrc/host_ppo.inc
+++ b/fsrl_amd/csrc/host_ppo.inc
@@ -67,32 +67,56 @@
     c->t_fwdbwd_ms = 0; c->n_fwdbwd = 0; c->k_ev_used = 0;
     CtrlBlock init{INT_MAX, 0, 0.0, 0.0f, 0.0f};
     *c->h_ctrl = init;
+    *reinterpret_cast<int*>(c->h_up + upload_layout(0, 0, 0).miss_count) = 0;
     hipStream_t s = c->compute;
-    HIPCHK(hipMemcpyAsync(c->ctrl, c->h_ctrl, sizeof(CtrlBlock), hipMemcpyHostToDevice, s));
     c->clip_fuse_active = false;
+    c->vnext_reuse_active = false;
     c->clip_perms.clear();
-    if (n == 0) { c->batch_ready = true; return 0; }
-    rc = clip_fuse_begin(c);
-    if (rc) return rc;
+    if (n == 0) {
+        HIPCHK(hipMemcpyAsync(c->d_up, c->h_up, UPLOAD_HEAD, hipMemcpyHostToDevice, s));
+        c->batch_ready = true;
+        return 0;
+    }
     int nseg = 0;
     c->h_seg[nseg++] = 0;
     for (int64_t i = 0; i + 1 < n; ++i) if (c->h_end[i]) c->h_seg[nseg++] = (int)i + 1;
     c->h_seg[nseg] = (int)n;
+    split_plan((int)n, batch_size, c->mb_start, c->mb_size);
+    const int bs_rows = (int)std::min<int64_t>(batch_size, std::max<int64_t>(n, 1));
+    rc = c->lay ? lay_ensure_mb(c, bs_rows) : ensure_ppo_buffers(c, bs_rows);
+    if (rc) return rc;
+    const size_t nmb = c->mb_start.size();
+    const UploadLayout u = upload_layout((size_t)n, (size_t)nseg, nmb);
+    memcpy(c->h_up + u.end, c->h_end, (size_t)n);
+    memcpy(c->h_up + u.seg, c->h_seg, (size_t)(nseg + 1) * 4);
+    memcpy(c->h_up + u.mb_start, c->mb_start.data(), nmb * 4);
+    memcpy(c->h_up + u.mb_size, c->mb_size.data(), nmb * 4);
+    c->d_end = reinterpret_cast<uint8_t*>(c->d_up + u.end); c->d_seg = reinterpret_cast<int*>(c->d_up + u.seg);
+    c->d_mbstart = reinterpret_cast<int*>(c->d_up + u.mb_start); c->d_mbsize = reinterpret_cast<int*>(c->d_up + u.mb_size);
+    rc = clip_fuse_begin(c);
+    if (rc) return rc;
     HIPCHK(hipEventRecord(c->ev_a, s));
-    HIPCHK(hipMemcpyAsync(c->d_indices, c->h_indices, (size_t)n * 4, hipMemcpyHostToDevice, s));
-    HIPCHK(hipMemcpyAsync(c->d_end, c->h_end, (size_t)n, hipMemcpyHostToDevice, s));
-    HIPCHK(hipMemcpyAsync(c->d_seg, c->h_seg, (size_t)(nseg + 1) * 4, hipMemcpyHostToDevice, s));
+    HIPCHK(hipMemcpyAsync(c->d_up, c->h_up, u.total, hipMemcpyHostToDevice, s));
     const int Do = c->cfg.obs_dim, Da = c->cfg.act_dim;
+    const bool reuse = !c->no_vnext_reuse && !c->lay && c->cfg.algo == FSRL_ALGO_PPO_LAG && c->cfg.n_critics >= 1;
     {
         const size_t work = (size_t)n * (2 * Do + Da + 1);
         const int blocks = (int)std::min<size_t>(2048, (work + 255) / 256);
-        hipLaunchKernelGGL(batch_gather_kernel, dim3(blocks), dim3(256), 0, s, c->st, c->b, c->d_indices,
-                           c->d_end, (int)n, Do, Da);
+        if (reuse) {
+            const int fblocks = (int)((n + 255) / 256);
+            hipLaunchKernelGGL(batch_gather_flag_kernel, dim3(blocks + fblocks), dim3(256), 0, s, c->st, c->b, c->d_indices,
+                               c->d_end, (int)n, Do, Da, blocks, NextSamePtrs{c->next_same, c->miss_list, c->miss_count});
+        } else {
+            hipLaunchKernelGGL(batch_gather_kernel, dim3(blocks), dim3(256), 0, s, c->st, c->b, c->d_indices,
+                               c->d_end, (int)n, Do, Da);
+        }
         HIPCHK(hipGetLastError());
     }
+    c->vnext_reuse_active = reuse;
     InferArgs ia{};
     ia.obs = c->b.obs; ia.obs_next = c->b.obs_next; ia.act = c->b.act; ia.flags = c->b.flags;
     ia.values = c->values; ia.vnext = c->vnext; ia.logp_old = c->logp_old; ia.mu_out = nullptr;
+    if (reuse) { ia.next_same = c->next_same; ia.miss_list = c->miss_list; ia.miss_count = c->miss_count; }
     if (c->cfg.algo == FSRL_ALGO_FOCOPS) {
         if (!c->mu_old) {
             HIPCHK(c->mem.dev(&c->mu_old, (size_t)c->alloc_rows * Da * 4));
@@ -108,20 +132,6 @@
     rc = launch_gae(c);
     if (rc) return rc;
     HIPCHK(hipEventRecord(c->ev_b, s));
-    split_plan((int)n, batch_size, c->mb_start, c->mb_size);
-    const int bs_rows = (int)std::min<int64_t>(batch_size, std::max<int64_t>(n, 1));
-    rc = c->lay ? lay_ensure_mb(c, bs_rows) : ensure_ppo_buffers(c, bs_rows);
-    if (rc) return rc;
-    const size_t nmb = c->mb_start.size();
-    if (nmb > c->mb_cap) {
-        HIPCHK(hipStreamSynchronize(s));
-        const size_t cap = nmb * 2;
-        HIPCHK(c->mem.regrow(c->mb_cap, nmb, cap, {Mem::D(&c->d_mbstart, cap * 4), Mem::D(&c->d_mbsize, cap * 4), Mem::H(&c->h_mbplan, cap * 2 * 4)}));
-    }
-    memcpy(c->h_mbplan, c->mb_start.data(), nmb * 4);
-    memcpy(c->h_mbplan + c->mb_cap, c->mb_size.data(), nmb * 4);
-    HIPCHK(hipMemcpyAsync(c->d_mbstart, c->h_mbplan, nmb * 4, hipMemcpyHostToDevice, s));
-    HIPCHK(hipMemcpyAsync(c->d_mbsize, c->h_mbplan + c->mb_cap, nmb * 4, hipMemcpyHostToDevice, s));
     c->batch_ready = true;
     return 0;
 }
@@ -155,6 +165,7 @@
     ia.obs = c->b.obs; ia.obs_next = c->b.obs_next; ia.act = nullptr; ia.flags = c->b.flags;
     ia.values = c->values; ia.vnext = c->vnext; ia.logp_old = nullptr; ia.mu_out = nullptr;
     ia.N = (int)c->N; ia.C = C; ia.max_action = c->cfg.max_action;
+    if (c->vnext_reuse_active) { ia.next_same = c->next_same; ia.miss_list = c->miss_list; ia.miss_count = c->miss_count; }
     int rc = launch_infer(c, ia, 2 * C, c->compute);
     if (rc) return rc;
     return launch_gae(c);
@@ -415,10 +426,8 @@
         HIPCHK(c->mem.dev(&c->clip_slots, (size_t)1024 * CLIP_SLOT_STRIDE * sizeof(unsigned long long)));
         HIPCHK(hipMemsetAsync(c->clip_slots, 0, (size_t)1024 * CLIP_SLOT_STRIDE * sizeof(unsigned long long), s));
     }
-    if (!c->clip_snap) HIPCHK(c->mem.dev(&c->clip_snap, ((size_t)c->n_alloc + 2 * (size_t)c->n_dev) * 4));
-    HIPCHK(hipMemcpyAsync(c->clip_snap, c->P, (size_t)c->n_alloc * 4, hipMemcpyDeviceToDevice, s));
-    HIPCHK(hipMemcpyAsync(c->clip_snap + c->n_alloc, c->M, (size_t)c->n_dev * 4, hipMemcpyDeviceToDevice, s));
-    HIPCHK(hipMemcpyAsync(c->clip_snap + c->n_alloc + c->n_dev, c->V, (size_t)c->n_dev * 4, hipMemcpyDeviceToDevice, s));
+    if (!c->clip_snap) HIPCHK(c->mem.dev(&c->clip_snap, c->pmv_bytes));
+    HIPCHK(hipMemcpyAsync(c->clip_snap, c->pmv, c->pmv_bytes, hipMemcpyDeviceToDevice, s));
     c->clip_snap_adam_t = c->adam_t;
     c->clip_fuse_active = true;
     return 0;
@@ -429,9 +438,7 @@
     const ClipFuseReplay rp = clip_fuse_replay_plan(c->clip_snap_adam_t, c->pass_index);
     c->clip_fuse_active = false; c->clip_fuse_dead = true;
     c->clip_fuse_fallbacks += 1;
-    HIPCHK(hipMemcpyAsync(c->P, c->clip_snap, (size_t)c->n_alloc * 4, hipMemcpyDeviceToDevice, s));
-    HIPCHK(hipMemcpyAsync(c->M, c->clip_snap + c->n_alloc, (size_t)c->n_dev * 4, hipMemcpyDeviceToDevice, s));
-    HIPCHK(hipMemcpyAsync(c->V, c->clip_snap + c->n_alloc + c->n_dev, (size_t)c->n_dev * 4, hipMemcpyDeviceToDevice, s));
+    HIPCHK(hipMemcpyAsync(c->pmv, c->clip_snap, c->pmv_bytes, hipMemcpyDeviceToDevice, s));
     c->adam_t = rp.adam_t; c->n_steps = rp.n_steps; c->pass_index = rp.pass_index;
     c->k_ev_used = 0;
     CtrlBlock init{INT_MAX, 0, 0.0, 0.0f, 0.0f};
@@ -468,6 +475,21 @@
     }
     out[0] = (c->clip_fuse_mode != 0 && !c->no_clip_fuse && !c->clip_fuse_dead) ? 1 : 0;
     out[1] = c->clip_fuse_fallbacks; out[2] = c->clip_fuse_steps; out[3] = c->clip_fuse_active ? 1 : 0;
+    return 0;
+}
+
+extern "C" int fsrl_ppo_process_stats(fsrl_ctx* c, int64_t* out) {
+    CHECK_ARG(c && out, "null argument");
+    if (!c->batch_ready) return fail(FSRL_ESTATE, "no batch: call fsrl_ppo_begin first");
+    ENTER_DEV(c);
+    out[0] = 0; out[1] = c->N; out[2] = 1; out[3] = c->vnext_reuse_active ? 1 : 0;
+    if (!c->vnext_reuse_active || c->N == 0) return 0;
+    int m = 0;
+    HIPCHK(hipStreamSynchronize(c->compute));
+    HIPCHK(hipMemcpy(&m, c->miss_count, sizeof(int), hipMemcpyDeviceToHost));
+    const int tiles = (int)((c->N + 15) / 16), jobs_y = 2 * c->cfg.n_critics + 1;
+    const InferSplit sp = infer_split(infer_grid_x(tiles, c->n_cus, jobs_y), jobs_y, c->cfg.n_critics, tiles, (m + 15) / 16);
+    out[0] = c->N - m; out[1] = m; out[2] = sp.equal;
     return 0;
 }
 
diff --git a/fsrl_amd/csrc/kernels_misc.hpp b/fsrl_amd/csrc/kernels_misc.hpp
--- a/fsrl_amd/csrc/kernels_misc.hpp
+++ b/fsrl_amd/csrc/kernels_misc.hpp
@@ -32,11 +32,11 @@
     float* obs; float* obs_next; float* act; double* rew; double* cost; uint8_t* flags;
 };
 
-__global__ void batch_gather_kernel(StorePtrs st, BatchPtrs b, const int* __restrict__ indices,
-                                    const uint8_t* __restrict__ end_flag, int n, int Do, int Da) {
+__device__ __forceinline__ void batch_gather_body(const StorePtrs& st, const BatchPtrs& b, const int* __restrict__ indices,
+                                                  const uint8_t* __restrict__ end_flag, int n, int Do, int Da, int bx, int nb) {
     const int per = 2 * Do + Da + 1;
-    for (size_t e = (size_t)blockIdx.x * blockDim.x + threadIdx.x; e < (size_t)n * per;
-         e += (size_t)gridDim.x * blockDim.x) {
+    for (size_t e = (size_t)bx * blockDim.x + threadIdx.x; e < (size_t)n * per;
+         e += (size_t)nb * blockDim.x) {
         const int row = (int)(e / per), f = (int)(e - (size_t)row * per);
         const size_t src = (size_t)indices[row];
         if (f < Do) b.obs[(size_t)row * Do + f] = st.obs[src * Do + f];
@@ -46,6 +46,45 @@
             b.rew[row] = st.rew[src];
             b.cost[row] = st.cost[src];
             b.flags[row] = (uint8_t)((st.flags[src] & 3) | (end_flag[row] ? 4 : 0));
+        }
+    }
+}
+__global__ void batch_gather_kernel(StorePtrs st, BatchPtrs b, const int* __restrict__ indices,
+                                    const uint8_t* __restrict__ end_flag, int n, int Do, int Da) {
+    batch_gather_body(st, b, indices, end_flag, n, Do, Da, (int)blockIdx.x, (int)gridDim.x);
+}
+
+struct NextSamePtrs { uint8_t* next_same; int* miss_list; int* miss_count; };
+__global__ __launch_bounds__(256) void batch_gather_flag_kernel(StorePtrs st, BatchPtrs b, const int* __restrict__ indices,
+                                                                const uint8_t* __restrict__ end_flag, int n, int Do, int Da,
+                                                                int gather_blocks, NextSamePtrs ns) {
+    if ((int)blockIdx.x < gather_blocks) {
+        batch_gather_body(st, b, indices, end_flag, n, Do, Da, (int)blockIdx.x, gather_blocks);
+        return;
+    }
+    const int fb = (int)blockIdx.x - gather_blocks, nfb = (int)gridDim.x - gather_blocks, lane = threadIdx.x & 63;
+    const uint32_t* __restrict__ so = reinterpret_cast<const uint32_t*>(st.obs);
+    const uint32_t* __restrict__ sn = reinterpret_cast<const uint32_t*>(st.obs_next);
+    for (int r0 = fb * 256; r0 < n; r0 += nfb * 256) {
+        const int r = r0 + (int)threadIdx.x;
+        bool miss = false;
+        if (r < n) {
+            miss = true;
+            if (r + 1 < n) {
+                const uint32_t* __restrict__ x = sn + (size_t)indices[r] * Do;
+                const uint32_t* __restrict__ y = so + (size_t)indices[r + 1] * Do;
+                uint32_t d = 0;
+                for (int k = 0; k < Do; ++k) d |= x[k] ^ y[k];
+                miss = d != 0;
+            }
+            ns.next_same[r] = miss ? 0 : 1;
+        }
+        const unsigned long long m = __ballot(miss);
+        if (m) {
+            int base = 0;
+            if (lane == __ffsll((long long)m) - 1) base = atomicAdd(ns.miss_count, __popcll(m));
+            base = __shfl(base, __ffsll((long long)m) - 1, 64);
+            if (miss) ns.miss_list[base + __popcll(m & ((1ull << lane) - 1ull))] = r;
         }
     }
 }
diff --git a/fsrl_amd/csrc/kernels_mlp.hpp b/fsrl_amd/csrc/kernels_mlp.hpp
--- a/fsrl_amd/csrc/kernels_mlp.hpp
+++ b/fsrl_amd/csrc/kernels_mlp.hpp
@@ -1,6 +1,7 @@
 #pragma once
 #include <type_traits>
 #include "common.hpp"
+#include "host_decisions.hpp"
 
 __host__ __device__ constexpr int tile_rows(int R) { return R > 16 ? R : 16; }
 
@@ -349,6 +350,9 @@
     float* sigma_param_out;
     unsigned* done;
     unsigned seq;
+    const uint8_t* next_same;
+    const int* miss_list;
+    const int* miss_count;
 };
 
 #define LOG_SQRT_2PI 0.9189385332046727f
@@ -360,34 +364,54 @@
     constexpr int NT = TileGeom<H>::NT;
     constexpr int NX = TileStage<H>::NX;
     const int tid = threadIdx.x;
-    const int job = blockIdx.y;
     const int C = a.C;
+    int job = blockIdx.y, bx = blockIdx.x, gx = gridDim.x;
+    int n_rows = a.N;
+    const int* __restrict__ list = nullptr;
+    if (a.next_same) {
+        const int m = *a.miss_count;
+        const InferSplit sp = infer_split((int)gridDim.x, (int)gridDim.y, C, (a.N + 15) >> 4, (m + 15) >> 4);
+        const int lb = (int)(blockIdx.y * gridDim.x + blockIdx.x), nb = C * sp.bn;
+        if (lb < nb) { job = C + lb / sp.bn; bx = lb % sp.bn; gx = sp.bn; list = a.miss_list; n_rows = m; }
+        else {
+            const int f = (lb - nb) / sp.bf;
+            if (f >= (int)gridDim.y - C) return;
+            bx = (lb - nb) % sp.bf; gx = sp.bf; job = f < C ? f : 2 * C;
+        }
+    }
     const bool is_actor = (job == 2 * C);
     const int net = is_actor ? 0 : 1 + (C > 0 ? job % C : 0);
     const bool use_next = (!is_actor) && job >= C;
     const NetOff no = md.net[net];
     const int Do = md.Do;
-    const int n_tiles = (a.N + 15) >> 4;
+    const int n_tiles = (n_rows + 15) >> 4;
     const unsigned magic = div_magic(Do);
     const float* __restrict__ X = use_next ? a.obs_next : a.obs;
-    int tile = blockIdx.x;
+    int tile = bx;
     int row0 = tile * 16;
-    int n_valid = min(16, a.N - row0);
+    int n_valid = min(16, n_rows - row0);
+    auto xload = [&](const int e, const int r0, const int nv) -> float {
+        if (e >= nv * Do) return 0.0f;
+        if (!list) return X[(size_t)r0 * Do + e];
+        const int i = div_by_magic((unsigned)e, magic), k = e - i * Do;
+        return X[(size_t)list[r0 + i] * Do + k];
+    };
     TileStage<H> stg;
-    stg.issue(P, no, Do, md.Da, X + (size_t)row0 * Do, nullptr, n_valid, tid);
+    stg.issue(P, no, Do, md.Da, list ? X : X + (size_t)row0 * Do, nullptr, list ? 0 : n_valid, tid);
+    if (list) {
+#pragma unroll
+        for (int u = 0; u < NX; ++u) stg.xv[u] = xload(tid + u * NT, row0, n_valid);
+    }
     FwdW2Frag<H> wf;
     wf.load(P + no.W2f, tid >> 6, tid & 63);
     stg.commit(sm, no, Do, tid);
     while (true) {
-        const int ntile = tile + gridDim.x;
-        const int nrow0 = ntile * 16, nn_valid = min(16, a.N - nrow0);
+        const int ntile = tile + gx;
+        const int nrow0 = ntile * 16, nn_valid = min(16, n_rows - nrow0);
         float xn[NX];
         if (ntile < n_tiles) {
 #pragma unroll
-            for (int u = 0; u < NX; ++u) {
-                const int e = tid + u * NT;
-                xn[u] = (e < nn_valid * Do) ? X[(size_t)nrow0 * Do + e] : 0.0f;
-            }
+            for (int u = 0; u < NX; ++u) xn[u] = xload(tid + u * NT, nrow0, nn_valid);
         }
         __syncthreads();
         tile_forward<H>(sm, P, no, Do, tid, wf);
@@ -398,7 +422,7 @@
                 a.raw_out[(size_t)(row0 + i) * a.raw_cols + o] = sm.out[i * FSRL_MAX_ACT + o];
             }
         } else if (tid < n_valid) {
-            const int r = row0 + tid;
+            const int r = list ? list[row0 + tid] : row0 + tid;
             if (!is_actor) {
                 float v = sm.out[tid * FSRL_MAX_ACT];
                 const int c = (C > 0) ? job % C : 0;
@@ -407,6 +431,7 @@
                     a.vnext[(size_t)c * a.N + r] = v;
                 } else {
                     a.values[(size_t)c * a.N + r] = v;
+                    if (a.next_same && r > 0 && a.next_same[r - 1]) a.vnext[(size_t)c * a.N + r - 1] = (a.flags[r - 1] & 1) ? 0.0f : v;
                 }
             } else {
                 float logp = 0.0f;
diff --git a/fsrl_amd/engine.py b/fsrl_amd/engine.py
--- a/fsrl_amd/engine.py
+++ b/fsrl_amd/engine.py
@@ -498,6 +498,11 @@
         _lib.check(self.lib.fsrl_ppo_clip_fuse_stats(self._ctx, out, C.byref(gn)))
         return dict(available=bool(out[0]), fallbacks=int(out[1]), steps=int(out[2]), last_update_fused=bool(out[3]),
                     grad_norm=np.float32(gn.value))
+
+    def ppo_process_stats(self):
+        out = (C.c_int64 * 4)()
+        _lib.check(self.lib.fsrl_ppo_process_stats(self._ctx, out))
+        return dict(rows_reused=int(out[0]), rows_evaluated=int(out[1]), equal_split=bool(out[2]), reuse=bool(out[3]))
 
     def ppo_update(self, lagrangians, rescaling, batch_size, repeat, perms=None, seed=0):
         n = self.ppo_begin(lagrangians, rescaling, batch_size)
diff --git a/include/fsrl_hip.h b/include/fsrl_hip.h
--- a/include/fsrl_hip.h
+++ b/include/fsrl_hip.h
@@ -155,6 +155,8 @@
 
 int fsrl_ppo_set_clip_fuse(fsrl_ctx* ctx, int32_t mode, int32_t limit_ticks);
 int fsrl_ppo_clip_fuse_stats(fsrl_ctx* ctx, int64_t* out, float* grad_norm_out);
+
+int fsrl_ppo_process_stats(fsrl_ctx* ctx, int64_t* out);
 
 typedef struct fsrl_group fsrl_group;
 int fsrl_group_create(fsrl_ctx** ctxs, int32_t k, fsrl_group** out);
```

Result: faster. 144.1 updates/s (median of 6 runs) (+1.6%).
